# fdrmrc/fictitious_domain_AL_preconditioners

Measured on AMD Instinct MI355X. Metric: FGMRES iterations/sec to 1e-8 residual, 3D Stokes-immersed (AL-preconditioned), higher is better.
Workload: dtype f64

## Files before the change

### fictitious_domain_al_preconditioners_amd/csrc/alfd.hip

```cpp

#include <hip/hip_runtime.h>
#include <rccl/rccl.h>

#include <algorithm>
#include <atomic>
#include <chrono>
#include <cmath>
#include <cstdio>
#include <cstdlib>
#include <cstring>
#include <memory>
#include <climits>
#include <condition_variable>
#include <functional>
#include <limits>
#include <mutex>
#include <string>
#include <thread>
#include <unordered_set>
#include <vector>

#include "alfd/alfd.h"
#include "kernels.hpp"
#include "kernels_vs.hpp"
// ... 157 lines not shown
  alfd_host_alltoallv_fn host_alltoallv = nullptr;
  void *host_user = nullptr;
  std::vector<char> host_send, host_recv;
  std::vector<std::vector<int64_t>> part;
  int nblocks = 0;
  int64_t n[ALFD_MAX_BLOCKS] = {0, 0, 0};
  int64_t off[ALFD_MAX_BLOCKS + 1] = {0, 0, 0, 0};
  int64_t nmax = 0;
  int64_t diag_cap = 0;
  DevCsr mat[ALFD_NSLOTS + 1];
  double *diag[ALFD_NDIAGS] = {nullptr, nullptr};
  int64_t diag_n[ALFD_NDIAGS] = {0, 0};
  alfd_config cfg;
  bool configured = false, is_setup = false;
  double *sc = nullptr;
  double *sc_host = nullptr;
  double *partial = nullptr;
  int64_t pstride = 0;
  double *gather = nullptr;
  double *dinv_aug = nullptr, *dA = nullptr, *s_aug = nullptr;
  double *dinv_a22 = nullptr, *dinv_aug2 = nullptr;
  double lam_max[7] = {0, 0, 0, 0, 0, 0, 0};
  double *dinv_k = nullptr;
  double *dinv_m = nullptr, *m_tmp = nullptr, *m_tmp2 = nullptr;
  double *n_r = nullptr, *n_z = nullptr, *n_p = nullptr, *n_Ap = nullptr;
  double *n_sc = nullptr, *n_sc_host = nullptr, *n_partial = nullptr, *n_gather = nullptr;
  int64_t mass_its = 0;
  int n_owner = 0;
  double *gd_bx = nullptr, *gd_q = nullptr;
  int nmp_group = 16;
  int nmp_host_stepped = 0;
  struct Spectrum {
    DevCsr own_Cs, own_Cts;
    DevCsr *Cs = nullptr, *Cts = nullptr;
    int64_t m = 0;
    double *t = nullptr, *ones = nullptr, *x = nullptr, *coef = nullptr, *linf = nullptr;
    int64_t coef_cap = 0;
    std::vector<void *> owned;
    std::vector<double> alpha, beta;
    bool have = false;
  } spec;
  int spec_group = 16;
  int spec_host_stepped = 0;
  HostCsr h_M, h_K;
  struct Hierarchy {
    std::vector<int32_t> agg[ALFD_MAX_LEVELS];
    std::vector<double> wgt[ALFD_MAX_LEVELS];
    int64_t ncoarse[ALFD_MAX_LEVELS] = {0, 0, 0, 0, 0, 0, 0, 0};
    HostCsr P[ALFD_MAX_LEVELS];
    DevCsr inv;
    std::vector<MlLevel> ml;
    TailTable *tail_tab = nullptr;
    bool built_partitioned = false;
    void clear_input() {
      for (int l = 0; l < ALFD_MAX_LEVELS; ++l) agg[l].clear(), wgt[l].clear(), P[l] = HostCsr(), ncoarse[l] = 0;
      built_partitioned = false;
    }
  } hier[2];
  struct Patch {
    bool on = false;
    int64_t m = 0, mpad = 0;
    DevCsr Ass, As, Ats, Cs, Cts;
    int32_t *S = nullptr;
    double *dinv = nullptr, *rS = nullptr, *zS = nullptr, *uS = nullptr, *eS = nullptr, *cd = nullptr,
           *cres = nullptr, *ctmp = nullptr, *rr = nullptr;
    double lmax = 0;
    uint8_t *tail_mask = nullptr;
    bool rep = false;
    int64_t m_loc = 0, piece = 1, lam_piece = 1;
    std::vector<int64_t> soff;
    DevCsr Cts_loc, Ctg;
    double *send = nullptr, *stage = nullptr, *lam_send = nullptr, *lam_stage = nullptr, *loc = nullptr;
  } patch;
  struct StrengthGraph {
    bool have = false, on_device = false;
    int64_t n_nodes = 0, node0 = 0;
    std::vector<int64_t> gp;
    std::vector<int32_t> gc, fixed;
    std::vector<double> gw, d;
  } sg;
  int ml_rep_level = -1;
  bool dots_replicated = false;
  int64_t ml_rep_threshold = 300000;
  int ml_fuse = 1;
  int ml_tail_rows = 0;
  int ml_gpu_galerkin = 1;
  double *g_w = nullptr, *g_tlam = nullptr;
  std::vector<int64_t> ml_coff[ALFD_MAX_LEVELS];
  const int64_t *up_col_offsets = nullptr;
  bool up_local_only = false;
  DevCsr rat_mat;
  double *rt_r = nullptr, *rt_z = nullptr, *rt_p = nullptr, *rt_Ap = nullptr, *rt_x = nullptr;
  double *rt_dinv = nullptr, *rt_partial = nullptr, *rt_scb = nullptr, *rt_coef = nullptr;
  double *rt_scb_host = nullptr;
  int64_t rational_its = 0;
  int64_t wmax = 0;
  std::vector<void *> ws_allocs;
  double *w_r = nullptr, *w_z = nullptr, *w_p = nullptr, *w_Ap = nullptr;
  double *c_d = nullptr, *c_res = nullptr, *c_tmp = nullptr;
  double *t_lam = nullptr;
  double *q_tmp = nullptr, *rhs_tmp = nullptr;
  double *V = nullptr, *Z = nullptr, *xb = nullptr, *bb = nullptr, *io = nullptr;
  double *st_in = nullptr, *st_out = nullptr;
  double lambda_max = 0, lambda_min = 0;
  int64_t inner_its = 0, mp_its = 0;
  int64_t inner_its_op[3] = {0, 0, 0};
  int inner_failures = 0, precond_applications = 0;
  std::vector<double> history;
  int timing = 0;
  std::vector<TimedLaunch> timed;
  double t_ms[ALFD_T_NCLASSES] = {0, 0, 0, 0};
  int64_t t_launches[ALFD_T_NCLASSES] = {0, 0, 0, 0};
  double t_bytes[ALFD_T_NCLASSES] = {0, 0, 0, 0};
  double t_fbytes[ALFD_T_NCLASSES] = {0, 0, 0, 0};
  double setup_s[ALFD_SETUP_NPHASES] = {0, 0, 0, 0, 0, 0, 0, 0};
  bool upload_since_setup = false;
  std::vector<void *> allocs;
  int spmv_stream_R = 2, spmv_stream_U = 8, spmv_nt = 0, spmv_grid_mult = 8;
  int spmv_group_R = 4, spmv_group_U = 4;
  bool vi_off = false;
  int vi_rows_R = 4, vi_rows_J = 2;
  int vi_xcd = 0;
  int vi_levels = 1;
  int vi_batched = 1;
  int win_RB_vi = 96;
  int win_vi = 1;
  int win_short_scale = 2;
  int vs_enable = 1, vs_NW = 4, vs_RB = 96, vs_xcd = 0, vs_share = 1, vs_wide = 1;
  int vs_lds_base_ok = -1;
  std::vector<int64_t> rb_ptr[ALFD_NSLOTS + 1];
  std::vector<int32_t> rb_rows[ALFD_NSLOTS + 1];
  int win_short_min_blocks = 256;
  int win_min_blocks = 256;
  int win_enable = 1, win_RB = 96, win_maxW = 4096, win_gap = 8, win_xcd = 0;
  int64_t ntot() const { return off[nblocks]; }
};

struct alfd_local_group {
  int n = 0;
  std::mutex mu;
  std::condition_variable cv;
  int arrived = 0;
  long generation = 0;
  std::vector<const void *> buf;
  std::vector<const int64_t *> off;
  void barrier() {
    std::unique_lock<std::mutex> lk(mu);
    const long g = generation;
    if (++arrived == n) {
      arrived = 0;
      ++generation;
      cv.notify_all();
    } else {
      cv.wait(lk, [&] { return generation != g; });
    }
  }
};

namespace alfd {

static int comm_allgather(alfd_ctx *ctx, const void *send, void *recv, size_t bytes) {
  if (ctx->local) {
    alfd_local_group *g = ctx->local;
    HIPC(hipStreamSynchronize(ctx->stream));
    g->buf[ctx->rank] = send;
    g->barrier();
    for (int p = 0; p < g->n; ++p)
// ... 107 lines not shown
}

static inline int grid_for_rows(int64_t nrows, int L) {
  const int64_t groups = (nrows + (kBlock / L) - 1) / (kBlock / L);
  return (int)std::max<int64_t>(1, std::min<int64_t>(groups, 256 * 8));
}

struct Timer {
  alfd_ctx *ctx;
  int cls;
  hipEvent_t a = nullptr, b = nullptr;
  bool on;
  Timer(alfd_ctx *c, int cl, double bytes, double fbytes = -1.0) : ctx(c), cls(cl) {
    on = ctx->timing >= 2 || (ctx->timing == 1 && cl == ALFD_T_SPMV_A);
    if (on) {
      hipEventCreate(&a);
      hipEventCreate(&b);
      hipEventRecord(a, ctx->stream);
      ctx->t_bytes[cls] += bytes;
      ctx->t_fbytes[cls] += fbytes < 0.0 ? bytes : fbytes;
      ctx->t_launches[cls]++;
    }
  }
  ~Timer() {
    if (on) {
      hipEventRecord(b, ctx->stream);
      ctx->timed.push_back({cls, a, b});
    }
  }
};

struct PhaseClock {
  alfd_ctx *ctx;
  int phase;
  std::chrono::steady_clock::time_point t0 = std::chrono::steady_clock::now();
  PhaseClock(alfd_ctx *c, int ph) : ctx(c), phase(ph) {}
  ~PhaseClock() {
    hipStreamSynchronize(ctx->stream);
    ctx->setup_s[phase] += std::chrono::duration<double>(std::chrono::steady_clock::now() - t0).count();
  }
};

static void flush_timers(alfd_ctx *ctx) {
  for (auto &t : ctx->timed) {
    hipEventSynchronize(t.b);
    float ms = 0;
    hipEventElapsedTime(&ms, t.a, t.b);
    ctx->t_ms[t.cls] += ms;
    hipEventDestroy(t.a);
    hipEventDestroy(t.b);
  }
  ctx->timed.clear();
}

template <int L>
static void launch_spmv_L(alfd_ctx *ctx, const DevCsr &m, const double *x, double *y, int epi, double alpha,
                          const double *d, double *y2) {
  const int grid = grid_for_rows(m.n_list, L);
  const double *xh = m.halo;
#define ALFD_SPMV(EPI, SP)                                                                          \
  hipLaunchKernelGGL((spmv_kernel<L, EPI, SP>), dim3(grid), dim3(kBlock), 0, ctx->stream, m.n_list, \
                     m.rp, m.col, m.val, m.rows, x, xh, m.n_local_cols, y, alpha, d, y2)
  if (m.sparse) {
    if (epi == 0) ALFD_SPMV(0, true);
    else if (epi == 1) ALFD_SPMV(1, true);
    else if (epi == 2) ALFD_SPMV(2, true);
    else ALFD_SPMV(3, true);
  } else {
    if (epi == 0) ALFD_SPMV(0, false);
    else if (epi == 1) ALFD_SPMV(1, false);
    else if (epi == 2) ALFD_SPMV(2, false);
    else ALFD_SPMV(3, false);
  }
#undef ALFD_SPMV
}

template <int R, int U, bool NT>
static void launch_stream(alfd_ctx *ctx, const DevCsr &m, const double *x, double *y, int epi, double alpha,
                          const double *d, double *y2) {
  const int64_t nbatches = (m.nrows + R - 1) / R;
  const int grid = (int)std::max<int64_t>(1, std::min<int64_t>((nbatches + 3) / 4, 256 * ctx->spmv_grid_mult));
#define ALFD_STREAM(EPI)                                                                              \
  hipLaunchKernelGGL((spmv_stream_kernel<R, U, EPI, NT>), dim3(grid), dim3(kBlock), 0, ctx->stream,   \
                     m.nrows, m.rp, m.col, m.val, x, m.halo, m.n_local_cols, y, alpha, d, y2)
  if (epi == 0) ALFD_STREAM(0);
  else if (epi == 1) ALFD_STREAM(1);
  else if (epi == 2) ALFD_STREAM(2);
  else ALFD_STREAM(3);
#undef ALFD_STREAM
}

template <bool NT>
static bool launch_stream_RU(alfd_ctx *ctx, const DevCsr &m, const double *x, double *y, int epi,
                             double alpha, const double *d, double *y2) {
  const int R = ctx->spmv_stream_R, U = ctx->spmv_stream_U;
#define ALFD_RU(RR, UU) \
  if (R == RR && U == UU) return launch_stream<RR, UU, NT>(ctx, m, x, y, epi, alpha, d, y2), true
  ALFD_RU(2, 2); ALFD_RU(2, 4); ALFD_RU(4, 2); ALFD_RU(4, 4); ALFD_RU(4, 8); ALFD_RU(8, 4); ALFD_RU(8, 8);
  ALFD_RU(1, 4); ALFD_RU(2, 8); ALFD_RU(8, 2);
#undef ALFD_RU
  return false;
}

template <int R, int U>
static void launch_window(alfd_ctx *ctx, const DevCsr &m, const double *x, double *y, int epi, double alpha,
                          const double *d, double *y2) {
  const size_t lds = (size_t)(m.win_maxW + (m.vi && !ctx->vi_off ? kDictMaxEntries : 0)) * sizeof(double);
#define ALFD_WIN(EPI, TAG)                                                                              \
  hipLaunchKernelGGL((spmv_window_kernel<R, U, EPI, TAG>), dim3((unsigned)m.win_nblocks), dim3(kBlock), \
                     lds, ctx->stream, m.nrows, m.win_RB, m.rp, m.col, m.lcol, m.val, m.blk_seg_begin,   \
                     m.blk_W, m.seg_col, m.seg_off, x, m.halo, m.n_local_cols, y, alpha, d, y2, ctx->win_xcd)
  const bool vi = m.vi && !ctx->vi_off;
  if (vi && ctx->vi_batched && m.vib_tab) {
#define ALFD_VIB(EPI, TAG)                                                                                    \
  hipLaunchKernelGGL((spmv_window_vib_kernel<EPI, TAG>), dim3((unsigned)m.win_nblocks), dim3(kBlock), lds,   \
                     ctx->stream, m.nrows, m.win_RB, m.rp, m.col, m.lcol, m.val, m.blk_seg_begin, m.blk_W,    \
                     m.seg_col, m.seg_off, x, m.halo, m.n_local_cols, y, alpha, d, y2, m.vidx, m.vidw,        \
                     m.blk_dict_off, m.blk_dict_n, m.dict, m.win_maxW, m.vib_tab, m.vib_cnt, m.vib_stride,    \
                     ctx->vi_xcd)
    if (m.tag == 0) {
      if (epi == 0) ALFD_VIB(0, 0);
      else if (epi == 1) ALFD_VIB(1, 0);
      else if (epi == 2) ALFD_VIB(2, 0);
      else ALFD_VIB(3, 0);
    } else {
      if (epi == 0) ALFD_VIB(0, 1);
      else if (epi == 1) ALFD_VIB(1, 1);
      else if (epi == 2) ALFD_VIB(2, 1);
      else ALFD_VIB(3, 1);
    }
#undef ALFD_VIB
    return;
  }
  if (vi && ctx->vi_rows_R > 0) {
    const int RR = ctx->vi_rows_R, JJ = ctx->vi_rows_J;
#define ALFD_VI(RV, JV, EPI)                                                                                  \
  hipLaunchKernelGGL((spmv_window_vi_kernel<RV, JV, EPI>), dim3((unsigned)m.win_nblocks), dim3(kBlock), lds,  \
                     ctx->stream, m.nrows, m.win_RB, m.rp, m.col, m.lcol, m.val, m.blk_seg_begin, m.blk_W,     \
                     m.seg_col, m.seg_off, x, m.halo, m.n_local_cols, y, alpha, d, y2, m.vidx, m.vidw, \
                     m.blk_dict_off, m.blk_dict_n, m.dict, m.win_maxW)
#define ALFD_VI_E(RV, JV)              \
  if (RR == RV && JJ == JV) {          \
    if (epi == 0) ALFD_VI(RV, JV, 0);  \
    else if (epi == 1) ALFD_VI(RV, JV, 1); \
    else if (epi == 2) ALFD_VI(RV, JV, 2); \
    else ALFD_VI(RV, JV, 3);           \
    return;                            \
  }
    ALFD_VI_E(4, 3) ALFD_VI_E(2, 4) ALFD_VI_E(4, 4)
    if (epi == 0) ALFD_VI(4, 2, 0);
    else if (epi == 1) ALFD_VI(4, 2, 1);
    else if (epi == 2) ALFD_VI(4, 2, 2);
    else ALFD_VI(4, 2, 3);
    return;
#undef ALFD_VI_E
#undef ALFD_VI
  }
  if (m.tag == 0) {
    if (epi == 0) ALFD_WIN(0, 0);
    else if (epi == 1) ALFD_WIN(1, 0);
    else if (epi == 2) ALFD_WIN(2, 0);
    else ALFD_WIN(3, 0);
  } else {
    if (epi == 0) ALFD_WIN(0, 1);
    else if (epi == 1) ALFD_WIN(1, 1);
    else if (epi == 2) ALFD_WIN(2, 1);
    else ALFD_WIN(3, 1);
  }
#undef ALFD_WIN
}

template <int L, int R, int U>
static void launch_window_group(alfd_ctx *ctx, const DevCsr &m, const double *x, double *y, int epi,
                                double alpha, const double *d, double *y2) {
  const size_t lds = (size_t)m.win_maxW * sizeof(double);
#define ALFD_WING(EPI, TAG)                                                                               \
  hipLaunchKernelGGL((spmv_window_group_kernel<L, R, U, EPI, TAG>), dim3((unsigned)m.win_nblocks),       \
                     dim3(kBlock), lds, ctx->stream, m.nrows, m.win_RB, m.rp, m.col, m.lcol, m.val,        \
                     m.blk_seg_begin, m.blk_W, m.seg_col, m.seg_off, x, m.halo, m.n_local_cols, y, alpha, \
                     d, y2)
  if (m.tag == 0) {
    if (epi == 0) ALFD_WING(0, 0);
    else if (epi == 1) ALFD_WING(1, 0);
    else if (epi == 2) ALFD_WING(2, 0);
    else ALFD_WING(3, 0);
  } else {
    if (epi == 0) ALFD_WING(0, 1);
    else if (epi == 1) ALFD_WING(1, 1);
    else if (epi == 2) ALFD_WING(2, 1);
    else ALFD_WING(3, 1);
  }
#undef ALFD_WING
}

template <int L>
static bool launch_window_group_RU(alfd_ctx *ctx, const DevCsr &m, const double *x, double *y, int epi,
                                   double alpha, const double *d, double *y2) {
  const int R = ctx->spmv_group_R, U = ctx->spmv_group_U;
#define ALFD_RU(RR, UU) \
  if (R == RR && U == UU) return launch_window_group<L, RR, UU>(ctx, m, x, y, epi, alpha, d, y2), true
  ALFD_RU(4, 4); ALFD_RU(2, 4); ALFD_RU(4, 2); ALFD_RU(8, 4); ALFD_RU(8, 2);
#undef ALFD_RU
  return false;
}

static bool launch_window_RU(alfd_ctx *ctx, const DevCsr &m, const double *x, double *y, int epi,
                             double alpha, const double *d, double *y2) {
  if (m.L == 32) return launch_window_group_RU<32>(ctx, m, x, y, epi, alpha, d, y2);
  if (m.L == 16) return launch_window_group_RU<16>(ctx, m, x, y, epi, alpha, d, y2);
  if (m.L == 8) return launch_window_group_RU<8>(ctx, m, x, y, epi, alpha, d, y2);
  if (m.L != 64) return false;
  const int R = ctx->spmv_stream_R, U = ctx->spmv_stream_U;
#define ALFD_RU(RR, UU) \
  if (R == RR && U == UU) return launch_window<RR, UU>(ctx, m, x, y, epi, alpha, d, y2), true
  ALFD_RU(1, 4); ALFD_RU(2, 4); ALFD_RU(2, 8); ALFD_RU(4, 2); ALFD_RU(4, 4); ALFD_RU(4, 8); ALFD_RU(8, 4);
  ALFD_RU(1, 8); ALFD_RU(1, 16); ALFD_RU(2, 16);
#undef ALFD_RU
  return false;
}


template <int L>
static void launch_vss(alfd_ctx *ctx, const DevCsr &m, const double *x, double *y, int epi, double alpha,
                       const double *d, double *y2) {
  const DevCsr::Vs &v = m.vs;
  const size_t lds = (size_t)kVsWinOff + (size_t)v.maxW * sizeof(double);
#define ALFD_VSS(EPI, TAG)                                                                                          \
  hipLaunchKernelGGL((spmv_vss_kernel<L, EPI, TAG>), dim3((unsigned)v.nb), dim3(256), lds, ctx->stream, v.stream, \
                     v.sb, v.tab, v.cnt, v.stride, v.seg_begin, v.blkW, v.seg_col, v.seg_off, v.doff, v.dn, v.dict, \
                     x, m.halo, m.n_local_cols, y, alpha, d, y2)
  if (m.tag == 0) {
    if (epi == 0) ALFD_VSS(0, 0);
    else if (epi == 1) ALFD_VSS(1, 0);
    else if (epi == 2) ALFD_VSS(2, 0);
    else ALFD_VSS(3, 0);
  } else {
    if (epi == 0) ALFD_VSS(0, 1);
    else if (epi == 1) ALFD_VSS(1, 1);
    else if (epi == 2) ALFD_VSS(2, 1);
    else ALFD_VSS(3, 1);
  }
#undef ALFD_VSS
}

static bool launch_vs(alfd_ctx *ctx, const DevCsr &m, const double *x, double *y, int epi, double alpha,
                      const double *d, double *y2, int64_t first_block = 0, int64_t n_blocks = -1) {
  const DevCsr::Vs &v = m.vs;
  if (ctx->vs_lds_base_ok < 0) {
    uint32_t *probe = nullptr, base = 1;
    if (hipMalloc((void **)&probe, sizeof(uint32_t)) == hipSuccess) {
      hipLaunchKernelGGL(vs_lds_base_probe_kernel, dim3(1), dim3(64), 4096, ctx->stream, probe);
      hipMemcpyAsync(&base, probe, sizeof(uint32_t), hipMemcpyDeviceToHost, ctx->stream);
      hipStreamSynchronize(ctx->stream);
      hipFree(probe);
    }
    ctx->vs_lds_base_ok = base == 0 ? 1 : 0;
    if (!ctx->vs_lds_base_ok)
      std::fprintf(stderr, "[alfd] dynamic LDS does not start at offset 0 (%u): batch-major SpMV formats disabled\n", base);
  }
  if (!ctx->vs_lds_base_ok) return false;
  if (v.L == 32) return launch_vss<32>(ctx, m, x, y, epi, alpha, d, y2), true;
  if (v.L == 16) return launch_vss<16>(ctx, m, x, y, epi, alpha, d, y2), true;
  if (v.L == 8) return launch_vss<8>(ctx, m, x, y, epi, alpha, d, y2), true;
  const int NW = ctx->vs_NW;
  const size_t lds = (size_t)(v.wide ? VsFmt<1>::kWinOff : VsFmt<0>::kWinOff) + (size_t)v.maxW * sizeof(double);
  if (n_blocks < 0) n_blocks = v.nb - first_block;
  if (n_blocks <= 0) return true;
  const unsigned grid = (unsigned)n_blocks;
  const int32_t base = (int32_t)first_block;
#define ALFD_VS_ARGS \
  v.stream, v.tab, v.stride, v.hdrb, v.segx, v.seg_stride, v.dict, x, m.halo, m.n_local_cols, y, alpha, d, y2, ctx->vs_xcd, base
#define ALFD_VS(EPI, NWV)                                                                                        \
  do {                                                                                                           \
    if (v.wide)                                     \
      hipLaunchKernelGGL((spmv_vs_kernel<EPI, 0, 4, 1>), dim3(grid), dim3(256), lds, ctx->stream,     \
                         ALFD_VS_ARGS);                                                                          \
    else if (m.tag == 0)                                                                                         \
      hipLaunchKernelGGL((spmv_vs_kernel<EPI, 0, NWV>), dim3(grid), dim3(64 * NWV), lds, ctx->stream, \
                         ALFD_VS_ARGS);                                                                          \
    else                \
      hipLaunchKernelGGL((spmv_vs_kernel<EPI, 1, 4>), dim3(grid), dim3(256), lds, ctx->stream,        \
                         ALFD_VS_ARGS);                                                                          \
  } while (0)
#define ALFD_VS_E(NWV)                  \
  do {                                  \
    if (epi == 0) ALFD_VS(0, NWV);      \
    else if (epi == 1) ALFD_VS(1, NWV); \
    else if (epi == 2) ALFD_VS(2, NWV); \
    else ALFD_VS(3, NWV);               \
  } while (0)
  if (NW == 8) ALFD_VS_E(8);
  else if (NW == 2) ALFD_VS_E(2);
  else ALFD_VS_E(4);
#undef ALFD_VS_E
#undef ALFD_VS
#undef ALFD_VS_ARGS
  return true;
}

static int halo_exchange(alfd_ctx *ctx, DevCsr &m, const double *x, hipStream_t st = nullptr);
static int spmv_launch_local(alfd_ctx *ctx, DevCsr &m, const double *x, double *y, int epi, double alpha, const double *d,
                             double *y2);

static int spmv_m(alfd_ctx *ctx, DevCsr &m, int cls, const double *x, double *y, int epi, double alpha = 0.0,
                  const double *d = nullptr, double *y2 = nullptr) {
  if (!m.present) return ctx->err = "matrix not set", ALFD_E_NOT_SETUP;
  const bool exchange = ctx->nranks > 1 && !m.rep && (ctx->local || ctx->host_alltoallv || m.n_halo > 0 || m.send_off.back() > 0);
  const bool overlap = exchange && (ctx->overlap_halo > 0 || (ctx->overlap_halo < 0 && (ctx->local || ctx->host_alltoallv))) && ctx->xstream && m.vs.on && m.vs.L == 64 && ctx->vs_enable && !ctx->vi_off &&
                       m.vs.nb_interior > 0 && !m.sparse && m.n_list > 0;
  if (overlap) {
    Timer tm(ctx, cls, m.algorithmic_bytes(), m.streamed_bytes(true, true));
    HIPC(hipEventRecord(ctx->ev_x, ctx->stream));
    if (!launch_vs(ctx, m, x, y, epi, alpha, d, y2, 0, m.vs.nb_interior)) return ctx->err = "batch-major launch failed", ALFD_E_HIP;
    HIPC(hipStreamWaitEvent(ctx->xstream, ctx->ev_x, 0));
    RC(halo_exchange(ctx, m, x, ctx->xstream));
    HIPC(hipEventRecord(ctx->ev_halo, ctx->xstream));
    HIPC(hipStreamWaitEvent(ctx->stream, ctx->ev_halo, 0));
    launch_vs(ctx, m, x, y, epi, alpha, d, y2, m.vs.nb_interior, m.vs.nb - m.vs.nb_interior);
    HIPC(hipGetLastError());
    return ALFD_OK;
  }
  if (exchange) RC(halo_exchange(ctx, m, x));
  if (m.sparse && epi != 1) {
    HIPC(hipMemsetAsync(y, 0, m.nrows * sizeof(double), ctx->stream));
    if (epi == 3) HIPC(hipMemsetAsync(y2, 0, m.nrows * sizeof(double), ctx->stream));
  }
  if (m.n_list == 0) return ALFD_OK;
  Timer tm(ctx, cls, m.algorithmic_bytes(), m.streamed_bytes(!ctx->vi_off, ctx->vs_enable != 0 && !ctx->vi_off));
  return spmv_launch_local(ctx, m, x, y, epi, alpha, d, y2);
}

static int spmv_launch_local(alfd_ctx *ctx, DevCsr &m, const double *x, double *y, int epi, double alpha, const double *d,
                             double *y2) {
  if (m.vs.on && ctx->vs_enable && !ctx->vi_off && launch_vs(ctx, m, x, y, epi, alpha, d, y2)) {
    HIPC(hipGetLastError());
    return ALFD_OK;
  }
  if (m.win && launch_window_RU(ctx, m, x, y, epi, alpha, d, y2)) {
    HIPC(hipGetLastError());
    return ALFD_OK;
  }
  if (m.L == 64 && !m.sparse && ctx->spmv_stream_R > 0) {
    const bool ok = ctx->spmv_nt ? launch_stream_RU<true>(ctx, m, x, y, epi, alpha, d, y2)
                                 : launch_stream_RU<false>(ctx, m, x, y, epi, alpha, d, y2);
    if (ok) {
      HIPC(hipGetLastError());
      return ALFD_OK;
    }
  }
  switch (m.L) {
    case 4: launch_spmv_L<4>(ctx, m, x, y, epi, alpha, d, y2); break;
    case 8: launch_spmv_L<8>(ctx, m, x, y, epi, alpha, d, y2); break;
    case 16: launch_spmv_L<16>(ctx, m, x, y, epi, alpha, d, y2); break;
    case 32: launch_spmv_L<32>(ctx, m, x, y, epi, alpha, d, y2); break;
    default: launch_spmv_L<64>(ctx, m, x, y, epi, alpha, d, y2); break;
  }
  HIPC(hipGetLastError());
  return ALFD_OK;
}

static int pick_short_row_format(alfd_ctx *ctx, DevCsr &m) {
  if (!m.vs.on || m.vs.L == 64 || m.nnz < 20000000 || ctx->vi_off || !ctx->vs_enable || m.sparse) return ALFD_OK;
  double *x = nullptr, *y = nullptr;
  const int64_t nx = std::max<int64_t>(ctx->nranks > 1 && !m.rep ? m.n_local_cols : m.ncols, 1);
  HIPC(hipMalloc((void **)&x, nx * sizeof(double)));
  HIPC(hipMalloc((void **)&y, std::max<int64_t>(m.nrows, 1) * sizeof(double)));
  HIPC(hipMemsetAsync(x, 0, nx * sizeof(double), ctx->stream));
  hipEvent_t e0, e1;
  HIPC(hipEventCreate(&e0));
  HIPC(hipEventCreate(&e1));
  float t[2] = {0.f, 0.f};
  bool ok = true;
  for (int f = 0; f < 2 && ok; ++f) {
    for (int it = 0; it < 6 && ok; ++it) {
      if (it == 1) hipEventRecord(e0, ctx->stream);
      m.vs.on = f == 0;
      ok = spmv_launch_local(ctx, m, x, y, 0, 0.0, nullptr, nullptr) == ALFD_OK;
    }
    m.vs.on = true;
    hipEventRecord(e1, ctx->stream);
    hipEventSynchronize(e1);
    hipEventElapsedTime(&t[f], e0, e1);
  }
  hipEventDestroy(e0);
  hipEventDestroy(e1);
  hipFree(x);
  hipFree(y);
  HIPC(hipGetLastError());
  if (ok && t[1] < 0.9f * t[0]) {
    m.vs.on = false;
    if (ctx->cfg.log_level > 0 || std::getenv("ALFD_LOG_UPLOAD"))
      std::fprintf(stderr, "[alfd] short-row operator (%lld rows, %lld nnz): without the batch-major form %.3f ms, with it %.3f ms per launch "
                   "-> batch-major form dropped\n", (long long)m.nrows, (long long)m.nnz, t[1] / 5.0, t[0] / 5.0);
  }
  return ALFD_OK;
}

static int spmv(alfd_ctx *ctx, int slot, const double *x, double *y, int epi, double alpha = 0.0,
                const double *d = nullptr, double *y2 = nullptr) {
  DevCsr &m = ctx->mat[slot];
  if (!m.present) return ctx->err = "matrix slot " + std::to_string(slot) + " not set", ALFD_E_NOT_SETUP;
  return spmv_m(ctx, m, slot == ALFD_A ? ALFD_T_SPMV_A : ALFD_T_SPMV_OTHER, x, y, epi, alpha, d, y2);
}

static int finish_dots(alfd_ctx *ctx, int64_t nb, int count, int out, int fin) {
  if (ctx->nranks == 1 || ctx->dots_replicated) {
    hipLaunchKernelGGL(dot_final_kernel, dim3(count), dim3(kBlock), 0, ctx->stream, ctx->partial, nb,
                       ctx->pstride, ctx->sc, out, fin);
    HIPC(hipGetLastError());
    return ALFD_OK;
  }
  hipLaunchKernelGGL(dot_final_kernel, dim3(count), dim3(kBlock), 0, ctx->stream, ctx->partial, nb,
                     ctx->pstride, ctx->sc, (int)S_STAGE, (int)FIN_STORE);
  HIPC(hipGetLastError());
  RC(comm_allgather(ctx, ctx->sc + S_STAGE, ctx->gather, (size_t)count * sizeof(double)));
  const int tgt = fin == FIN_STORE ? out : (int)S_TMP;
  hipLaunchKernelGGL(rank_sum_kernel, dim3(1), dim3(64), 0, ctx->stream, ctx->gather, ctx->nranks, count,
                     ctx->sc, tgt);
  if (fin != FIN_STORE) {
    hipLaunchKernelGGL(dot_final_kernel, dim3(1), dim3(kBlock), 0, ctx->stream, ctx->sc + S_TMP,
                       (int64_t)1, (int64_t)0, ctx->sc, out, fin);
  }
  HIPC(hipGetLastError());
  return ALFD_OK;
}

static int dot_async(alfd_ctx *ctx, int64_t npad, const double *x, const double *y, int out,
                     int fin = FIN_STORE) {
  const int64_t nb = npad / kChunk;
  if (nb > 0) {
    Timer tm(ctx, ALFD_T_DOT, 16.0 * npad);
    hipLaunchKernelGGL(dot_partial_kernel, dim3((unsigned)nb), dim3(kBlock), 0, ctx->stream, x, y,
                       ctx->partial);
  }
  HIPC(hipGetLastError());
  return finish_dots(ctx, nb, 1, out, fin);
}

static int read_scalars(alfd_ctx *ctx, int first, int count) {
  hipLaunchKernelGGL(mirror_scalars_kernel, dim3(1), dim3(kBlock), 0, ctx->stream, ctx->sc + first,
                     ctx->sc_host + first, count);
  HIPC(hipGetLastError());
  HIPC(hipStreamSynchronize(ctx->stream));
  return ALFD_OK;
}

#define VEC_LAUNCH(kernel, npad, bytes_per_elem, ...)                                              \
  do {                                                                                             \
    if ((npad) > 0) {                                                                              \
      Timer tm__(ctx, ALFD_T_VEC, (double)(bytes_per_elem) * (double)(npad));                      \
      hipLaunchKernelGGL(kernel, dim3((unsigned)((npad) / kChunk)), dim3(kBlock), 0, ctx->stream,  \
                         __VA_ARGS__);                                                             \
    }                                                                                              \
  } while (0)

enum OpKind { OP_AUG = 0, OP_MP = 1, OP_A22 = 2, OP_AUG2 = 3, OP_K = 4, OP_MASS = 5, OP_CCT = 6 };

static inline int64_t op_npad(const alfd_ctx *ctx, int op) {
  if (op == OP_MASS || op == OP_CCT) return pad_chunk(ctx->n[ctx->nblocks - 1]);
  return (op == OP_AUG || op == OP_K) ? pad_chunk(ctx->n[0]) : op == OP_AUG2 ? ctx->off[2] : pad_chunk(ctx->n[1]);
}

static int winv_scale(alfd_ctx *ctx, double alpha, const double *src, double *dst);
static int nested_mp_solve(alfd_ctx *ctx, const double *b, double *x);

static inline bool gd_nested(const alfd_ctx *ctx) {
  return !ctx->cfg.grad_div_in_A && (ctx->cfg.variant == ALFD_AL_STOKES || ctx->cfg.variant == ALFD_AL_STOKES_DIAG);
}

static int op_apply(alfd_ctx *ctx, int op, const double *x, double *y, bool exact_w = false) {
  const double *w = ctx->diag[ALFD_INVW];
  switch (op) {
    case OP_AUG:
      RC(spmv(ctx, ALFD_A, x, y, 0));
      if (ctx->cfg.aug_assembled) return ALFD_OK;
      if (exact_w && ctx->cfg.w_inverse != ALFD_W_DIAGONAL) {
        RC(spmv(ctx, ALFD_C, x, ctx->t_lam, 0));
        RC(winv_scale(ctx, 1.0, ctx->t_lam, ctx->t_lam));
      } else {
        RC(spmv(ctx, ALFD_C, x, ctx->t_lam, 2, 0.0, w));
      }
      RC(spmv(ctx, ALFD_CT, ctx->t_lam, y, 1, ctx->cfg.gamma));
      if (!gd_nested(ctx)) return ALFD_OK;
      if (exact_w) {
        RC(spmv(ctx, ALFD_B, x, ctx->gd_bx, 0));
        RC(nested_mp_solve(ctx, ctx->gd_bx, ctx->gd_q));
      } else {
        RC(spmv(ctx, ALFD_B, x, ctx->gd_q, 2, 0.0, ctx->diag[ALFD_MP_LUMPED_INV]));
      }
      return spmv(ctx, ALFD_BT, ctx->gd_q, y, 1, ctx->cfg.gamma_grad_div);
    case OP_MASS:
      return spmv(ctx, ALFD_M, x, y, 0);
    case OP_CCT:
      RC(spmv_m(ctx, *ctx->spec.Cts, ALFD_T_SPMV_OTHER, x, ctx->spec.t, 0));
      return spmv_m(ctx, *ctx->spec.Cs, ALFD_T_SPMV_OTHER, ctx->spec.t, y, 0);
    case OP_MP:
      return spmv(ctx, ALFD_MP, x, y, 0);
    case OP_K:
      return spmv(ctx, ALFD_A, x, y, 0);
    case OP_A22:
      RC(spmv(ctx, ALFD_A2, x, y, 0));
      if (exact_w && ctx->cfg.w_inverse != ALFD_W_DIAGONAL) {
        RC(spmv(ctx, ALFD_M, x, ctx->t_lam, 0));
        RC(winv_scale(ctx, 1.0, ctx->t_lam, ctx->t_lam));
      } else {
        RC(spmv(ctx, ALFD_M, x, ctx->t_lam, 2, 0.0, w));
      }
      return spmv(ctx, ALFD_M, ctx->t_lam, y, 1, ctx->cfg.gamma2);
    default: {
      const double *x1 = x + ctx->off[1];
      double *y1 = y + ctx->off[1];
      const int64_t nlp = pad_chunk(ctx->n[2]);
      RC(spmv(ctx, ALFD_C, x, ctx->t_lam, 0));
      RC(spmv(ctx, ALFD_M, x1, ctx->t_lam, 1, -1.0));
      if (exact_w) RC(winv_scale(ctx, 1.0, ctx->t_lam, ctx->t_lam));
      else VEC_LAUNCH(pmul_scale_kernel, nlp, 24, 1.0, w, ctx->t_lam, ctx->t_lam);
      RC(spmv(ctx, ALFD_A, x, y, 0));
      RC(spmv(ctx, ALFD_CT, ctx->t_lam, y, 1, ctx->cfg.gamma));
      RC(spmv(ctx, ALFD_A2, x1, y1, 0));
      return spmv(ctx, ALFD_M, ctx->t_lam, y1, 1, -ctx->cfg.gamma2);
    }
  }
}

static const double *op_dinv(const alfd_ctx *ctx, int op) {
  return op == OP_AUG ? ctx->dinv_aug : op == OP_A22 ? ctx->dinv_a22 : op == OP_AUG2 ? ctx->dinv_aug2
         : op == OP_K ? ctx->dinv_k : op == OP_MASS ? ctx->dinv_m : ctx->diag[ALFD_MP_LUMPED_INV];
}

struct ChebCoef {
  double theta, delta, sigma, rho;
  ChebCoef(double lmax, double ratio) {
    const double lmin = lmax / ratio;
    theta = 0.5 * (lmax + lmin), delta = 0.5 * (lmax - lmin);
    sigma = theta / delta;
    rho = 1.0 / sigma;
  }
  void step(double &c1, double &c2) {
    const double rho_new = 1.0 / (2.0 * sigma - rho);
    c1 = rho_new * rho, c2 = 2.0 * rho_new / delta;
    rho = rho_new;
  }
};

template <class Apply>
static int cheb_sweep(alfd_ctx *ctx, int64_t npad, const double *dinv, double lmax, double ratio, int degree, double *cd,
                      double *cres, double *ctmp, const double *r, double *z, Apply apply) {
  ChebCoef k(lmax, ratio);
  VEC_LAUNCH(cheb_init_kernel, npad, degree > 1 ? 40 : 32, 1.0 / k.theta, dinv, r, cd, z, cres, degree > 1 ? 1 : 0);
  for (int j = 1; j < degree; ++j) {
    RC(apply(cd, ctmp));
    double c1, c2;
    k.step(c1, c2);
    VEC_LAUNCH(cheb_step_kernel, npad, 64, c1, c2, dinv, ctmp, cres, cd, z);
  }
  HIPC(hipGetLastError());
  return ALFD_OK;
}

static int cheb_apply(alfd_ctx *ctx, int op, const double *r, double *z, int64_t npad) {
  const int k = ctx->cfg.cheb_degree;
  if (k > 1) HIPC(hipMemsetAsync(ctx->c_tmp, 0, npad * sizeof(double), ctx->stream));
  return cheb_sweep(ctx, npad, op_dinv(ctx, op), ctx->lam_max[op], ctx->cfg.cheb_eig_ratio, k, ctx->c_d, ctx->c_res,
// ... 2401 lines not shown
    out.col.insert(out.col.end(), t_col[t].begin(), t_col[t].end());
    out.val.insert(out.val.end(), t_val[t].begin(), t_val[t].end());
  }
}

static int upload_matrix(alfd_ctx *ctx, int slot, int64_t nrows, int64_t ncols, const int64_t *rp,
                         const int32_t *col, const double *val);
static int upload_level(alfd_ctx *ctx, DevCsr &dst, const HostCsr &h) {
  static const int32_t no_col = 0;
  static const double no_val = 0;
  RC(upload_matrix(ctx, kScratchSlot, h.nrows, h.ncols, h.rp.data(), h.col.empty() ? &no_col : h.col.data(),
                   h.val.empty() ? &no_val : h.val.data()));
  csr_free(dst);
  dst = std::move(ctx->mat[kScratchSlot]);
  ctx->mat[kScratchSlot] = DevCsr();
  dst.tag = 1;
  return ALFD_OK;
}

struct AugOp {
  DevCsr *A = nullptr, *C = nullptr, *Ct = nullptr;
  int clsA = ALFD_T_SPMV_OTHER;
  const double *w = nullptr;
  double gamma = 0;
  double *tlam = nullptr;
  const uint8_t *mask = nullptr;
  int64_t npad = 0;
  const double *dinv = nullptr;
  double *cd = nullptr, *cres = nullptr, *ctmp = nullptr;
  double lmax = 0;
};

struct LevelView {
  AugOp op;
  double *r = nullptr, *z = nullptr, *t = nullptr;
  DevCsr *R = nullptr, *P = nullptr;
  double *rc = nullptr, *zc = nullptr;
};

static LevelView level_view(alfd_ctx *ctx, int h, int l) {
  MlLevel &L = ctx->hier[h].ml[l];
  const bool rep = h == 0 && ctx->ml_rep_level >= 0 && l >= ctx->ml_rep_level;
  LevelStore &S = rep ? L.rep : L.loc;
  LevelView V;
  AugOp &F = V.op;
  F.A = l > 0 ? &S.A : &ctx->mat[h == 0 ? ALFD_A : ALFD_A2];
  F.C = l > 0 ? &S.C : &ctx->mat[h == 0 ? ALFD_C : ALFD_M];
  F.Ct = l > 0 ? &S.Ct : &ctx->mat[h == 0 ? ALFD_CT : ALFD_M];
  F.clsA = l == 0 && h == 0 ? ALFD_T_SPMV_A : ALFD_T_SPMV_OTHER;
  F.w = rep ? ctx->g_w : ctx->diag[ALFD_INVW];
  F.gamma = h == 0 ? ctx->cfg.gamma : ctx->cfg.gamma2;
  F.tlam = rep ? ctx->g_tlam : ctx->t_lam;
  F.mask = L.tail_mask;
  F.npad = S.npad;
  F.dinv = S.dinv;
  F.cd = S.cd, F.cres = S.cres, F.ctmp = S.ctmp;
  F.lmax = L.lmax;
  V.r = S.r, V.z = S.z, V.t = S.t;
  if (l + 1 < (int)ctx->hier[h].ml.size()) {
    MlLevel &M = ctx->hier[h].ml[l + 1];
    LevelStore &N = rep ? M.rep : M.loc;
    V.R = &N.R, V.P = &N.P;
    V.rc = N.r, V.zc = N.z;
  }
  return V;
}

static AugOp patch_aug(alfd_ctx *ctx) {
  alfd_ctx::Patch &Q = ctx->patch;
  AugOp F;
  F.A = &Q.Ass, F.C = &Q.Cs, F.Ct = &Q.Cts;
  F.w = Q.rep ? ctx->g_w : ctx->diag[ALFD_INVW];
  F.tlam = Q.rep ? ctx->g_tlam : ctx->t_lam;
  F.gamma = ctx->cfg.gamma;
  F.mask = Q.tail_mask;
  F.npad = Q.mpad;
  F.dinv = Q.dinv;
  F.cd = Q.cd, F.cres = Q.cres, F.ctmp = Q.ctmp;
  F.lmax = Q.lmax;
  return F;
}

static int fused_AC(alfd_ctx *ctx, const AugOp &F, const double *x, double *y) {
  RC(spmv_m(ctx, *F.A, F.clsA, x, y, 0));
  return spmv_m(ctx, *F.C, ALFD_T_SPMV_OTHER, x, F.tlam, 2, 0.0, F.w);
}

static int aug_apply(alfd_ctx *ctx, const AugOp &F, const double *x, double *y) {
  if (ctx->cfg.aug_assembled) return spmv_m(ctx, *F.A, F.clsA, x, y, 0);
  RC(fused_AC(ctx, F, x, y));
  return spmv_m(ctx, *F.Ct, ALFD_T_SPMV_OTHER, F.tlam, y, 1, F.gamma);
}

static int aug_lambda_max(alfd_ctx *ctx, const AugOp &F, int64_t n, int64_t goff, double *v, double *wv, double *lmax) {
  if (n > 0)
    hipLaunchKernelGGL(hash_vector_kernel, dim3((unsigned)((n + 255) / 256)), dim3(256), 0, ctx->stream, n, goff, v);
  double lam = 0;
  RC(power_lambda(ctx, F.npad, F.dinv, v, wv, [&](const double *x, double *y) { return aug_apply(ctx, F, x, y); }, &lam));
  *lmax = lam * ctx->cfg.cheb_safety;
  HIPC(hipMemsetAsync(v, 0, F.npad * sizeof(double), ctx->stream));
  HIPC(hipMemsetAsync(wv, 0, F.npad * sizeof(double), ctx->stream));
  return ALFD_OK;
}


static bool plain_form(const alfd_ctx *ctx, const DevCsr &m) {
  return m.present && !m.vs.on && !m.win && !(m.L == 64 && !m.sparse && ctx->spmv_stream_R > 0);
}

static bool fused_ok(const alfd_ctx *ctx, const AugOp &F) {
  return ctx->ml_fuse && ctx->nranks == 1 && !ctx->cfg.aug_assembled && !gd_nested(ctx) &&
         ctx->cfg.w_inverse == ALFD_W_DIAGONAL && F.mask && F.A->present && F.C->present && plain_form(ctx, *F.Ct);
}

static int aug_tail(alfd_ctx *ctx, const AugOp &F, int mode, const AugTailArgs &p, double vec_bytes) {
  const DevCsr &m = *F.Ct;
  const int nb_rows = m.n_list > 0 ? grid_for_rows(m.n_list, m.L) : 0;
  const unsigned grid = (unsigned)nb_rows + (unsigned)(F.npad / kChunk);
  if (grid == 0) return ALFD_OK;
  Timer tm(ctx, ALFD_T_SPMV_OTHER, m.algorithmic_bytes() + vec_bytes * (double)F.npad,
           m.streamed_bytes(false) + vec_bytes * (double)F.npad);
#define ALFD_TAIL(LL, MM)                                                                                         \
  hipLaunchKernelGGL((aug_tail_kernel<LL, MM>), dim3(grid), dim3(kBlock), 0, ctx->stream, m.n_list, m.rp, m.col,  \
                     m.val, m.sparse ? m.rows : (const int32_t *)nullptr, F.tlam, nb_rows, F.mask, p)
#define ALFD_TAIL_L(LL)                                      \
  switch (mode) {                                            \
    case TAIL_STEP: ALFD_TAIL(LL, TAIL_STEP); break;         \
    case TAIL_LAST: ALFD_TAIL(LL, TAIL_LAST); break;         \
    case TAIL_LAST_ADD: ALFD_TAIL(LL, TAIL_LAST_ADD); break; \
    case TAIL_RES: ALFD_TAIL(LL, TAIL_RES); break;           \
    case TAIL_RES_INIT: ALFD_TAIL(LL, TAIL_RES_INIT); break; \
    default: ALFD_TAIL(LL, TAIL_RES_INIT_ADD); break;        \
  }
  switch (m.L) {
    case 4: ALFD_TAIL_L(4) break;
    case 8: ALFD_TAIL_L(8) break;
    case 16: ALFD_TAIL_L(16) break;
    case 32: ALFD_TAIL_L(32) break;
    default: ALFD_TAIL_L(64) break;
  }
#undef ALFD_TAIL_L
#undef ALFD_TAIL
  HIPC(hipGetLastError());
  return ALFD_OK;
}

static int cheb_fused(alfd_ctx *ctx, const AugOp &F, int degree, double ratio, const double *r, double *z, double *zout,
                      bool have_init) {
  ChebCoef k(F.lmax, ratio);
  if (!have_init) VEC_LAUNCH(cheb_init_z_kernel, F.npad, 24, 1.0 / k.theta, F.dinv, r, z);
  for (int j = 1; j < degree; ++j) {
    RC(fused_AC(ctx, F, j == 1 ? z : F.cd, F.ctmp));
    AugTailArgs p;
    k.step(p.c1, p.c2);
    p.gamma = F.gamma;
    p.dinv = F.dinv, p.y = F.ctmp, p.rin = j == 1 ? r : F.cres, p.din = j == 1 ? z : F.cd;
    p.res = F.cres, p.d = F.cd, p.z = z, p.zout = zout;
    const bool last = j == degree - 1;
    RC(aug_tail(ctx, F, !last ? TAIL_STEP : zout ? TAIL_LAST_ADD : TAIL_LAST, p, last && zout ? 88.0 : 64.0));
  }
  HIPC(hipGetLastError());
  return ALFD_OK;
}

static int aug_cheb(alfd_ctx *ctx, const AugOp &F, int degree, double ratio, const double *r, double *z) {
  if (fused_ok(ctx, F)) return cheb_fused(ctx, F, degree, ratio, r, z, nullptr, false);
  return cheb_sweep(ctx, F.npad, F.dinv, F.lmax, ratio, degree, F.cd, F.cres, F.ctmp, r, z,
                    [&](const double *x, double *y) { return aug_apply(ctx, F, x, y); });
}

static int fused_residual(alfd_ctx *ctx, const AugOp &F, const double *r, double *t) {
  AugTailArgs p;
  p.gamma = F.gamma, p.y = t, p.rin = r, p.res = t;
  return aug_tail(ctx, F, TAIL_RES, p, 24.0);
}

static int fused_correct(alfd_ctx *ctx, const AugOp &F, int degree, double ratio, const double *r, double *t, double *zc,
                         double *zout) {
  AugTailArgs p;
  p.gamma = F.gamma, p.c1 = 1.0 / ChebCoef(F.lmax, ratio).theta;
  p.dinv = F.dinv, p.y = t, p.rin = r, p.res = t, p.z = zc, p.zout = zout;
  p.store_res = degree > 1;
  if (degree <= 1 && zout) return aug_tail(ctx, F, TAIL_RES_INIT_ADD, p, 24.0 + 32.0 + 24.0);
  RC(aug_tail(ctx, F, TAIL_RES_INIT, p, 24.0 + (degree > 1 ? 40.0 : 32.0)));
  return cheb_fused(ctx, F, degree, ratio, t, zc, zout, true);
}

static int build_tail_mask(alfd_ctx *ctx, const DevCsr &m, int64_t npad, uint8_t **mask) {
  *mask = nullptr;
  if (ctx->nranks > 1 || !m.present || npad == 0 || m.nrows > npad) return ALFD_OK;
  double *q = nullptr;
  RC(ws_alloc_zero(ctx, &q, npad / 8));
  *mask = reinterpret_cast<uint8_t *>(q);
  if (m.n_list > 0)
    hipLaunchKernelGGL(mark_rows_kernel, dim3((unsigned)((m.n_list + 255) / 256)), dim3(256), 0, ctx->stream, m.n_list,
                       m.sparse ? m.rows : (const int32_t *)nullptr, *mask);
  HIPC(hipGetLastError());
  return ALFD_OK;
}

static_assert(kTailMaxLevels == ALFD_MAX_LEVELS + 1, "TailTable holds every level of a hierarchy");

static bool tail_form(const DevCsr &m) { return m.present && !m.vs.on && !m.win; }

static TailCsr tail_csr(const DevCsr &m) {
  TailCsr t;
  t.rp = m.rp, t.col = m.col, t.val = m.val, t.rows = m.sparse ? m.rows : nullptr;
  t.n_list = m.n_list, t.nrows = m.nrows;
  t.L = m.L, t.sparse = m.sparse ? 1 : 0;
  return t;
}

static int build_tail_table(alfd_ctx *ctx) {
  const alfd_config &c = ctx->cfg;
  alfd_ctx::Hierarchy &H = ctx->hier[1];
  const int last = (int)H.ml.size() - 1;
  std::vector<TailTable> tab(1);
  TailTable &T = tab[0];
  std::memset(&T, 0, sizeof(T));
  T.nlev = last + 1;
  T.has_inv = H.inv.present ? 1 : 0;
  if (H.inv.present) T.inv = tail_csr(H.inv);
  for (int l = 1; l <= last; ++l) {
    const LevelView V = level_view(ctx, 1, l);
    TailLevel &F = T.lev[l];
    F.A = tail_csr(*V.op.A), F.C = tail_csr(*V.op.C), F.Ct = tail_csr(*V.op.Ct);
    if (l < last) F.R = tail_csr(*V.R), F.P = tail_csr(*V.P);
    F.dinv = V.op.dinv, F.w = V.op.w, F.tlam = V.op.tlam;
    F.r = V.r, F.z = V.z, F.t = V.t, F.cd = V.op.cd, F.cres = V.op.cres, F.ctmp = V.op.ctmp;
    F.gamma = V.op.gamma, F.npad = V.op.npad;
    F.degree = l == last ? c.ml_coarse_degree : c.ml_smooth_degree_coarse > 0 ? c.ml_smooth_degree_coarse : c.ml_smooth_degree;
    ChebCoef k(V.op.lmax, l == last ? c.ml_coarse_ratio : c.ml_smooth_ratio);
    F.inv_theta = 1.0 / k.theta;
    for (int j = 1; j < F.degree && j <= kTailMaxDegree; ++j) k.step(F.c1[j - 1], F.c2[j - 1]);
  }
  double *q = nullptr;
  RC(ws_alloc_zero(ctx, &q, (int64_t)((sizeof(TailTable) + 7) / 8)));
  H.tail_tab = reinterpret_cast<TailTable *>(q);
  HIPC(hipMemcpyAsync(H.tail_tab, &T, sizeof(TailTable), hipMemcpyHostToDevice, ctx->stream));
  HIPC(hipStreamSynchronize(ctx->stream));
  return ALFD_OK;
}

static bool tail_ok(alfd_ctx *ctx, int l, const double *r, const double *z) {
  const alfd_config &c = ctx->cfg;
  alfd_ctx::Hierarchy &H = ctx->hier[1];
  const int last = (int)H.ml.size() - 1;
  if (!H.tail_tab || l < 1 || H.ml[l].loc.n > ctx->ml_tail_rows || r != H.ml[l].loc.r || z != H.ml[l].loc.z) return false;
  if (ctx->nranks != 1 || c.aug_assembled || c.w_inverse != ALFD_W_DIAGONAL) return false;
  const int sdeg = c.ml_smooth_degree_coarse > 0 ? c.ml_smooth_degree_coarse : c.ml_smooth_degree;
  if (sdeg - 1 > kTailMaxDegree || (!H.inv.present && c.ml_coarse_degree - 1 > kTailMaxDegree)) return false;
  if (H.inv.present && !tail_form(H.inv)) return false;
  for (int j = l; j <= last; ++j) {
    const LevelStore &L = H.ml[j].loc;
    if (!tail_form(L.A) || !tail_form(L.C) || !tail_form(L.Ct)) return false;
    if (j > l && (!tail_form(L.R) || !tail_form(L.P))) return false;
  }
  return true;
}

static int allgather_pieces(alfd_ctx *ctx, const double *mine, const std::vector<int64_t> &offs, int64_t piece, double *send,
                            double *stage, double *whole) {
  const int64_t n_me = offs[ctx->rank + 1] - offs[ctx->rank];
  if (n_me > 0) HIPC(hipMemcpyAsync(send, mine, n_me * sizeof(double), hipMemcpyDeviceToDevice, ctx->stream));
  RC(comm_allgather(ctx, send, stage, (size_t)piece * sizeof(double)));
  for (int p = 0; p < ctx->nranks; ++p) {
    const int64_t np = offs[p + 1] - offs[p];
    if (np > 0)
      HIPC(hipMemcpyAsync(whole + offs[p], stage + (int64_t)p * piece, np * sizeof(double), hipMemcpyDeviceToDevice, ctx->stream));
  }
  return ALFD_OK;
}

static int ml_cycle(alfd_ctx *ctx, int h, int l, const double *r, double *z) {
  const alfd_config &c = ctx->cfg;
  alfd_ctx::Hierarchy &H = ctx->hier[h];
  const int last = (int)H.ml.size() - 1;
  if (h == 1 && ctx->ml_tail_rows > 0 && tail_ok(ctx, l, r, z)) {
    Timer tm(ctx, ALFD_T_SPMV_OTHER, 0.0);
    hipLaunchKernelGGL(ml_tail_kernel, dim3(1), dim3(kTailBlock), 0, ctx->stream, H.tail_tab, l);
    HIPC(hipGetLastError());
    return ALFD_OK;
  }
  const LevelView L = level_view(ctx, h, l);
  const AugOp &F = L.op;
  if (l == last) {
// ... 9 lines not shown
  } else {
    RC(aug_apply(ctx, F, z, L.t));
    VEC_LAUNCH(sub_from_kernel, F.npad, 24, r, L.t);
  }
  RC(spmv_m(ctx, *L.R, ALFD_T_SPMV_OTHER, L.t, L.rc, 0));
  if (h == 0 && l + 1 == ctx->ml_rep_level) {
    MlLevel &N = H.ml[l + 1];
    RC(allgather_pieces(ctx, N.loc.r, N.offs, N.maxpiece, N.send, N.stage, N.rep.r));
    RC(ml_cycle(ctx, h, l + 1, N.rep.r, N.rep.z));
    RC(spmv_m(ctx, N.loc.P, ALFD_T_SPMV_OTHER, N.P_global_cols ? N.rep.z : N.rep.z + N.offs[ctx->rank], z, 1, 1.0));
  } else {
    RC(ml_cycle(ctx, h, l + 1, L.rc, L.zc));
    RC(spmv_m(ctx, *L.P, ALFD_T_SPMV_OTHER, L.zc, z, 1, 1.0));
  }
  if (fuse) {
    RC(fused_AC(ctx, F, z, L.t));
    RC(fused_correct(ctx, F, sdeg, c.ml_smooth_ratio, r, L.t, L.r, z));
    return ALFD_OK;
  }
  RC(aug_apply(ctx, F, z, L.t));
  VEC_LAUNCH(sub_from_kernel, F.npad, 24, r, L.t);
  RC(aug_cheb(ctx, F, sdeg, c.ml_smooth_ratio, L.t, L.r));
  VEC_LAUNCH(axpy_kernel, F.npad, 24, (const double *)nullptr, 0, 1.0, L.r, z);
  HIPC(hipGetLastError());
  return ALFD_OK;
}

static int ml_apply_rep(alfd_ctx *ctx, const double *r, double *z) {
  alfd_ctx::Patch &Q = ctx->patch;
  const int64_t n0p = pad_chunk(ctx->n[0]);
  const unsigned gm = (unsigned)std::max<int64_t>(1, (Q.m_loc + 255) / 256);
  const bool pen = !ctx->cfg.aug_assembled;
  const int last = ctx->nblocks - 1;
  const int64_t s0 = Q.soff[ctx->rank];
  const AugOp F = patch_aug(ctx);
  const int pdeg = ctx->cfg.ml_patch_degree;
  const double pratio = ctx->cfg.ml_patch_ratio;
  if (Q.m_loc > 0) hipLaunchKernelGGL(gather_kernel, dim3(gm), dim3(256), 0, ctx->stream, Q.m_loc, Q.S, r, Q.loc);
  RC(allgather_pieces(ctx, Q.loc, Q.soff, Q.piece, Q.send, Q.stage, Q.rS));
  RC(aug_cheb(ctx, F, pdeg, pratio, Q.rS, Q.zS));
  VEC_LAUNCH(scale_copy_kernel, n0p, 16, 1.0, r, Q.rr);
  RC(spmv_m(ctx, Q.Ats, ALFD_T_SPMV_OTHER, Q.zS, Q.rr, 1, -1.0));
  if (pen) {
    RC(spmv_m(ctx, Q.Cs, ALFD_T_SPMV_OTHER, Q.zS, ctx->g_tlam, 2, 0.0, ctx->g_w));
    RC(spmv_m(ctx, Q.Ctg, ALFD_T_SPMV_OTHER, ctx->g_tlam, Q.rr, 1, -ctx->cfg.gamma));
  }
  RC(ml_cycle(ctx, 0, 0, Q.rr, z));
  if (Q.m_loc > 0) hipLaunchKernelGGL(scatter_add_kernel, dim3(gm), dim3(256), 0, ctx->stream, Q.m_loc, Q.S, Q.zS + s0, z);
  RC(spmv_m(ctx, Q.As, ALFD_T_SPMV_OTHER, z, Q.loc, 0));
  if (pen) {
    RC(spmv(ctx, ALFD_C, z, ctx->t_lam, 2, 0.0, ctx->diag[ALFD_INVW]));
    RC(allgather_pieces(ctx, ctx->t_lam, ctx->part[last], Q.lam_piece, Q.lam_send, Q.lam_stage, ctx->g_tlam));
    RC(spmv_m(ctx, Q.Cts_loc, ALFD_T_SPMV_OTHER, ctx->g_tlam, Q.loc, 1, ctx->cfg.gamma));
  }
  RC(allgather_pieces(ctx, Q.loc, Q.soff, Q.piece, Q.send, Q.stage, Q.uS));
  VEC_LAUNCH(sub_from_kernel, Q.mpad, 24, Q.rS, Q.uS);
  RC(aug_cheb(ctx, F, pdeg, pratio, Q.uS, Q.eS));
  if (Q.m_loc > 0) hipLaunchKernelGGL(scatter_add_kernel, dim3(gm), dim3(256), 0, ctx->stream, Q.m_loc, Q.S, Q.eS + s0, z);
  HIPC(hipGetLastError());
  return ALFD_OK;
}

static int ml_apply(alfd_ctx *ctx, const double *r, double *z) {
  alfd_ctx::Patch &Q = ctx->patch;
  if (!Q.on) return ml_cycle(ctx, 0, 0, r, z);
  if (Q.rep) return ml_apply_rep(ctx, r, z);
  const int64_t n0p = pad_chunk(ctx->n[0]);
  const unsigned gm = (unsigned)((Q.m + 255) / 256);
  const bool pen = !ctx->cfg.aug_assembled;
  const double *w = ctx->diag[ALFD_INVW];
  const AugOp F = patch_aug(ctx);
  const int pdeg = ctx->cfg.ml_patch_degree;
  const double pratio = ctx->cfg.ml_patch_ratio;
  hipLaunchKernelGGL(gather_kernel, dim3(gm), dim3(256), 0, ctx->stream, Q.m, Q.S, r, Q.rS);
  RC(aug_cheb(ctx, F, pdeg, pratio, Q.rS, Q.zS));
  VEC_LAUNCH(scale_copy_kernel, n0p, 16, 1.0, r, Q.rr);
  RC(spmv_m(ctx, Q.Ats, ALFD_T_SPMV_OTHER, Q.zS, Q.rr, 1, -1.0));
  if (pen) {
    RC(spmv_m(ctx, Q.Cs, ALFD_T_SPMV_OTHER, Q.zS, ctx->t_lam, 2, 0.0, w));
    RC(spmv(ctx, ALFD_CT, ctx->t_lam, Q.rr, 1, -ctx->cfg.gamma));
  }
  RC(ml_cycle(ctx, 0, 0, Q.rr, z));
  hipLaunchKernelGGL(scatter_add_kernel, dim3(gm), dim3(256), 0, ctx->stream, Q.m, Q.S, Q.zS, z);
  RC(spmv_m(ctx, Q.As, ALFD_T_SPMV_OTHER, z, Q.uS, 0));
  if (fused_ok(ctx, F)) {
    RC(spmv(ctx, ALFD_C, z, ctx->t_lam, 2, 0.0, w));
    RC(fused_correct(ctx, F, pdeg, pratio, Q.rS, Q.uS, Q.eS, nullptr));
  } else {
    if (pen) {
      RC(spmv(ctx, ALFD_C, z, ctx->t_lam, 2, 0.0, w));
      RC(spmv_m(ctx, Q.Cts, ALFD_T_SPMV_OTHER, ctx->t_lam, Q.uS, 1, ctx->cfg.gamma));
    }
    VEC_LAUNCH(sub_from_kernel, Q.mpad, 24, Q.rS, Q.uS);
    RC(aug_cheb(ctx, F, pdeg, pratio, Q.uS, Q.eS));
  }
  hipLaunchKernelGGL(scatter_add_kernel, dim3(gm), dim3(256), 0, ctx->stream, Q.m, Q.S, Q.eS, z);
  HIPC(hipGetLastError());
  return ALFD_OK;
}

static void spgemm_host(const HostCsr &A, const HostCsr &Pm, HostCsr &out) {
  const int64_t nrows = A.nrows, nc = Pm.ncols;
  const int T = (int)std::max<int64_t>(1, std::min<int64_t>(std::min(16u, std::max(1u, std::thread::hardware_concurrency())),
                                                           (nrows + 4095) / 4096));
  std::vector<std::vector<int32_t>> t_cnt(T), t_col(T);
  std::vector<std::vector<double>> t_val(T);
  std::vector<std::thread> th;
  for (int t = 0; t < T; ++t)
    th.emplace_back([&, t]() {
      const int64_t i0 = nrows * t / T, i1 = nrows * (t + 1) / T;
      std::vector<int64_t> stamp(nc, -1);
      std::vector<double> acc(nc, 0.0);
      std::vector<int32_t> touched;
      t_cnt[t].reserve(i1 - i0);
      for (int64_t i = i0; i < i1; ++i) {
        touched.clear();
        for (int64_t k = A.rp[i]; k < A.rp[i + 1]; ++k) {
          const double a = A.val[k];
          const int64_t j = A.col[k];
          for (int64_t e = Pm.rp[j]; e < Pm.rp[j + 1]; ++e) {
            const int32_t J = Pm.col[e];
            if (stamp[J] != i) {
              stamp[J] = i;
              acc[J] = std::fma(a, Pm.val[e], 0.0);
              touched.push_back(J);
            } else {
              acc[J] = std::fma(a, Pm.val[e], acc[J]);
            }
          }
        }
        std::sort(touched.begin(), touched.end());
        t_cnt[t].push_back((int32_t)touched.size());
        for (int32_t J : touched) {
          t_col[t].push_back(J);
          t_val[t].push_back(acc[J]);
        }
      }
    });
  for (auto &x : th) x.join();
  out.nrows = nrows;
  out.ncols = nc;
  out.rp.assign(1, 0);
  out.rp.reserve(nrows + 1);
  int64_t total = 0;
  for (int t = 0; t < T; ++t) total += (int64_t)t_col[t].size();
  out.col.clear();
  out.val.clear();
  out.col.reserve(total);
  out.val.reserve(total);
  for (int t = 0; t < T; ++t) {
    for (int32_t c : t_cnt[t]) out.rp.push_back(out.rp.back() + c);
    out.col.insert(out.col.end(), t_col[t].begin(), t_col[t].end());
    out.val.insert(out.val.end(), t_val[t].begin(), t_val[t].end());
    std::vector<int32_t>().swap(t_col[t]);
    std::vector<double>().swap(t_val[t]);
  }
}

static void extract_host(const HostCsr &A, const std::vector<int32_t> &rows, const int32_t *colmap, int64_t ncols,
                         bool full_rows, HostCsr &out) {
  out.nrows = full_rows ? A.nrows : (int64_t)rows.size();
  out.ncols = ncols;
  out.rp.assign(out.nrows + 1, 0);
  out.col.clear();
  out.val.clear();
  int64_t next = 0;
  for (size_t q = 0; q < rows.size(); ++q) {
    const int64_t i = rows[q], orow = full_rows ? i : (int64_t)q;
    for (; next <= orow; ++next) out.rp[next] = (int64_t)out.col.size();
    for (int64_t k = A.rp[i]; k < A.rp[i + 1]; ++k) {
      const int32_t c = colmap ? colmap[A.col[k]] : A.col[k];
      if (c < 0) continue;
      out.col.push_back(c);
      out.val.push_back(A.val[k]);
    }
// ... 2247 lines not shown
    HIPC(hipMemcpyAsync(blocks[b], dev + ctx->off[b], ctx->n[b] * sizeof(double), hipMemcpyDeviceToHost,
                        ctx->stream));
  HIPC(hipStreamSynchronize(ctx->stream));
  return ALFD_OK;
}

static void reset_stats(alfd_ctx *ctx) {
  ctx->inner_its = ctx->mp_its = 0;
  ctx->inner_its_op[0] = ctx->inner_its_op[1] = ctx->inner_its_op[2] = 0;
  ctx->inner_failures = ctx->precond_applications = 0;
  ctx->rational_its = 0;
  ctx->mass_its = 0;
}
static void fill_result(alfd_ctx *ctx, alfd_result *res, int status) {
  res->status = status;
  res->inner_iterations = ctx->inner_its;
  res->mp_iterations = ctx->mp_its;
  res->inner_failures = ctx->inner_failures;
  res->precond_applications = ctx->precond_applications;
  res->lambda_max = ctx->lambda_max;
  res->rational_iterations = ctx->rational_its;
  res->mass_iterations = ctx->mass_its;
}

}

#define CHECK_CTX()                       \
  if (!ctx) return ALFD_E_INVALID;        \
  if (hipSetDevice(ctx->device) != hipSuccess) return ctx->err = "hipSetDevice failed", ALFD_E_HIP
#define CHECK_SETUP() \
  if (!ctx->is_setup) return ctx->err = "alfd_setup not called", ALFD_E_NOT_SETUP

extern "C" {

int alfd_abi_version(void) { return ALFD_ABI_VERSION; }

const char *alfd_strerror(int s) {
  switch (s) {
    case ALFD_OK: return "ok";
    case ALFD_E_INVALID: return "invalid argument";
    case ALFD_E_HIP: return "HIP runtime error";
    case ALFD_E_NO_CONVERGENCE_OUTER: return "FGMRES: no convergence (SolverControl::NoConvergence)";
    case ALFD_E_NO_CONVERGENCE_INNER: return "inner CG: no convergence (SolverControl::NoConvergence)";
    case ALFD_E_BREAKDOWN: return "breakdown (NaN residual)";
    case ALFD_E_NOT_SETUP: return "context not set up";
    case ALFD_E_COMM: return "RCCL error";
    case ALFD_E_UNSUPPORTED: return "not implemented";
    default: return "unknown status";
  }
}

const char *alfd_last_error(alfd_ctx_t ctx) { return ctx ? ctx->err.c_str() : "null context"; }

int alfd_create(alfd_ctx_t *out, int device_id) {
  if (!out) return ALFD_E_INVALID;
  *out = nullptr;
  int ndev = 0;
  if (hipGetDeviceCount(&ndev) != hipSuccess || ndev <= 0 || device_id < 0 || device_id >= ndev)
    return ALFD_E_HIP;
  if (hipSetDevice(device_id) != hipSuccess) return ALFD_E_HIP;
  alfd_ctx *ctx = new alfd_ctx;
  ctx->device = device_id;
  if (hipStreamCreateWithFlags(&ctx->xstream, hipStreamNonBlocking) != hipSuccess ||
      hipEventCreateWithFlags(&ctx->ev_x, hipEventDisableTiming) != hipSuccess ||
      hipEventCreateWithFlags(&ctx->ev_halo, hipEventDisableTiming) != hipSuccess)
    ctx->xstream = nullptr;
  if (const char *e = std::getenv("ALFD_SPMV_OVERLAP_HALO")) ctx->overlap_halo = std::atoi(e);
  if (hipStreamCreateWithFlags(&ctx->stream, hipStreamNonBlocking) != hipSuccess) {
    delete ctx;
    return ALFD_E_HIP;
  }
  alfd_default_config(&ctx->cfg, ALFD_AL_STOKES);
  if (const char *e = std::getenv("ALFD_SPMV_STREAM_R")) ctx->spmv_stream_R = std::atoi(e);
  if (const char *e = std::getenv("ALFD_SPMV_STREAM_U")) ctx->spmv_stream_U = std::atoi(e);
  if (const char *e = std::getenv("ALFD_SPMV_NT")) ctx->spmv_nt = std::atoi(e);
  if (const char *e = std::getenv("ALFD_SPMV_GRID")) ctx->spmv_grid_mult = std::max(1, std::atoi(e));
  if (const char *e = std::getenv("ALFD_SPMV_WINDOW")) ctx->win_enable = std::atoi(e);
  if (const char *e = std::getenv("ALFD_SPMV_WINDOW_RB")) ctx->win_RB = std::max(4, std::atoi(e));
  if (const char *e = std::getenv("ALFD_SPMV_WINDOW_MIN_BLOCKS")) ctx->win_min_blocks = std::max(1, std::atoi(e));
  if (const char *e = std::getenv("ALFD_SPMV_WINDOW_SHORT_MIN_BLOCKS")) ctx->win_short_min_blocks = std::max(1, std::atoi(e));
  if (const char *e = std::getenv("ALFD_SPMV_WINDOW_MAXW")) ctx->win_maxW = std::min(16384, std::max(256, std::atoi(e)));
  if (const char *e = std::getenv("ALFD_ML_REPLICATE")) ctx->ml_rep_threshold = std::atoll(e);
  if (const char *e = std::getenv("ALFD_ML_GPU_GALERKIN")) ctx->ml_gpu_galerkin = std::atoi(e);
  if (const char *e = std::getenv("ALFD_ML_FUSE")) ctx->ml_fuse = std::atoi(e) != 0;
  if (const char *e = std::getenv("ALFD_SPMV_VI_LEVELS")) ctx->vi_levels = std::atoi(e);
  if (const char *e = std::getenv("ALFD_SPMV_BATCH_MAJOR")) ctx->vs_enable = std::atoi(e);
  if (const char *e = std::getenv("ALFD_SPMV_BATCH_MAJOR_ROWS")) ctx->vs_RB = std::max(4, std::min(kVsMaxRows, std::atoi(e)));
  if (const char *e = std::getenv("ALFD_SPMV_VI_XCD")) ctx->vi_xcd = std::atoi(e);
  if (const char *e = std::getenv("ALFD_SPMV_VI_BATCHED")) ctx->vi_batched = std::atoi(e);
  if (const char *e = std::getenv("ALFD_SPMV_WINDOW_RB_VI")) ctx->win_RB_vi = std::atoi(e);
  if (const char *e = std::getenv("ALFD_SPMV_VI_R")) ctx->vi_rows_R = std::atoi(e);
  if (const char *e = std::getenv("ALFD_SPMV_VI_J")) ctx->vi_rows_J = std::atoi(e);
  if (const char *e = std::getenv("ALFD_SPMV_VALUE_INDEX")) ctx->win_vi = std::atoi(e);
  if (const char *e = std::getenv("ALFD_SPMV_GROUP_R")) ctx->spmv_group_R = std::atoi(e);
  if (const char *e = std::getenv("ALFD_SPMV_GROUP_U")) ctx->spmv_group_U = std::atoi(e);
  if (const char *e = std::getenv("ALFD_SPMV_WINDOW_SHORT")) ctx->win_short_scale = std::max(0, std::atoi(e));
  if (const char *e = std::getenv("ALFD_SPMV_WINDOW_GAP")) ctx->win_gap = std::max(1, std::atoi(e));
  if (const char *e = std::getenv("ALFD_SPMV_WINDOW_XCD")) ctx->win_xcd = std::atoi(e);
  *out = ctx;
  return ALFD_OK;
}

int alfd_destroy(alfd_ctx_t ctx) {
  if (!ctx) return ALFD_E_INVALID;
  hipSetDevice(ctx->device);
  hipStreamSynchronize(ctx->stream);
  flush_timers(ctx);
  free_levels(ctx);
  spectrum_release(ctx);
  csr_free(ctx->rat_mat);
  for (DevCsr &m : ctx->mat) csr_free(m);
  for (void *p : ctx->ws_allocs) hipFree(p);
  for (void *p : ctx->allocs) hipFree(p);
  if (ctx->sc_host) hipHostFree(ctx->sc_host);
  if (ctx->n_sc_host) hipHostFree(ctx->n_sc_host);
  if (ctx->rt_scb_host) hipHostFree(ctx->rt_scb_host);
  if (ctx->nccl) ncclCommDestroy(ctx->nccl);
  if (ctx->xstream) hipStreamDestroy(ctx->xstream);
  if (ctx->ev_x) hipEventDestroy(ctx->ev_x);
  if (ctx->ev_halo) hipEventDestroy(ctx->ev_halo);
  hipStreamDestroy(ctx->stream);
  delete ctx;
  return ALFD_OK;
}

int alfd_comm_unique_id(void *id_out, size_t bytes) {
  static_assert(sizeof(ncclUniqueId) <= ALFD_UNIQUE_ID_BYTES, "unique id size");
  if (!id_out || bytes < sizeof(ncclUniqueId)) return ALFD_E_INVALID;
  ncclUniqueId id;
  if (ncclGetUniqueId(&id) != ncclSuccess) return ALFD_E_COMM;
  std::memset(id_out, 0, bytes);
  std::memcpy(id_out, &id, sizeof(id));
  return ALFD_OK;
}

int alfd_comm_init(alfd_ctx_t ctx, int rank, int nranks, const void *id, size_t bytes) {
  CHECK_CTX();
  if (nranks < 1 || rank < 0 || rank >= nranks) return ALFD_E_INVALID;
  ctx->rank = rank;
  ctx->nranks = nranks;
  if (nranks == 1) return ALFD_OK;
  if (!id || bytes < sizeof(ncclUniqueId)) return ALFD_E_INVALID;
  ncclUniqueId uid;
  std::memcpy(&uid, id, sizeof(uid));
  if (ncclCommInitRank(&ctx->nccl, nranks, uid, rank) != ncclSuccess)
    return ctx->err = "ncclCommInitRank failed", ALFD_E_COMM;
  if (rank == 0) {
    int v = 0;
    if (ncclGetVersion(&v) == ncclSuccess) std::fprintf(stderr, "[alfd] RCCL version %d, %d ranks\n", v, nranks);
  }
  return ALFD_OK;
}

int alfd_local_group_create(int nranks, alfd_local_group **out) {
  if (!out || nranks < 1) return ALFD_E_INVALID;
  alfd_local_group *g = new alfd_local_group;
  g->n = nranks;
  g->buf.assign(nranks, nullptr);
  g->off.assign(nranks, nullptr);
  *out = g;
  return ALFD_OK;
}

int alfd_local_group_destroy(alfd_local_group *g) {
  if (!g) return ALFD_E_INVALID;
  delete g;
  return ALFD_OK;
// ... 974 lines not shown
                                                                    : fgmres(ctx, res);
  hipStreamSynchronize(ctx->stream);
  res->solve_seconds = std::chrono::duration<double>(std::chrono::steady_clock::now() - t0).count();
  flush_timers(ctx);
  fill_result(ctx, res, rc);
  return rc;
}

int alfd_download_solution(alfd_ctx_t ctx, double *const *x) {
  CHECK_CTX();
  CHECK_SETUP();
  if (!x) return ALFD_E_INVALID;
  return to_host(ctx, ctx->xb, x);
}

int alfd_solve(alfd_ctx_t ctx, const double *const *rhs, double *const *x, alfd_result *res) {
  CHECK_CTX();
  CHECK_SETUP();
  if (!rhs || !x || !res) return ALFD_E_INVALID;
  RC(alfd_upload_rhs(ctx, rhs, x));
  const int rc = alfd_solve_resident(ctx, res);
  const int rc2 = alfd_download_solution(ctx, x);
  return rc != ALFD_OK ? rc : rc2;
}

int alfd_get_history(alfd_ctx_t ctx, double *out, int32_t capacity, int32_t *count) {
  if (!ctx) return ALFD_E_INVALID;
  if (count) *count = (int32_t)ctx->history.size();
  if (out)
    for (int32_t i = 0; i < capacity && i < (int32_t)ctx->history.size(); ++i) out[i] = ctx->history[i];
  return ALFD_OK;
}

int alfd_spmv(alfd_ctx_t ctx, int slot, const double *x, double *y, int mode, double alpha) {
  CHECK_CTX();
  if (slot < 0 || slot >= ALFD_NSLOTS || !ctx->mat[slot].present) return ALFD_E_INVALID;
  if (!x || !y || (mode != 0 && mode != 1)) return ALFD_E_INVALID;
  const DevCsr &m = ctx->mat[slot];
  const int64_t nx = ctx->nranks > 1 ? (int64_t)m.n_local_cols : m.ncols;
  double *dx = nullptr, *dy = nullptr;
  HIPC(hipMalloc((void **)&dx, std::max<int64_t>(nx, 1) * sizeof(double)));
  HIPC(hipMalloc((void **)&dy, std::max<int64_t>(m.nrows, 1) * sizeof(double)));
  HIPC(hipMemcpyAsync(dx, x, nx * sizeof(double), hipMemcpyHostToDevice, ctx->stream));
  HIPC(hipMemcpyAsync(dy, y, m.nrows * sizeof(double), hipMemcpyHostToDevice, ctx->stream));
  const int rc = spmv(ctx, slot, dx, dy, mode, alpha);
  if (rc == ALFD_OK) {
    HIPC(hipMemcpyAsync(y, dy, m.nrows * sizeof(double), hipMemcpyDeviceToHost, ctx->stream));
    HIPC(hipStreamSynchronize(ctx->stream));
  }
  hipFree(dx);
  hipFree(dy);
  return rc;
}

int alfd_spmv_scaled(alfd_ctx_t ctx, int slot, const double *x, const double *d, double *y, double *y2) {
  CHECK_CTX();
  if (slot < 0 || slot >= ALFD_NSLOTS || !ctx->mat[slot].present) return ALFD_E_INVALID;
  if (!x || !d || !y || y2 == y) return ALFD_E_INVALID;
  const DevCsr &m = ctx->mat[slot];
  const int64_t nx = ctx->nranks > 1 ? (int64_t)m.n_local_cols : m.ncols;
  const size_t rows = std::max<int64_t>(m.nrows, 1) * sizeof(double), nb = m.nrows * sizeof(double);
  double *dx = nullptr, *dd = nullptr, *dy = nullptr, *dy2 = nullptr;
  HIPC(hipMalloc((void **)&dx, std::max<int64_t>(nx, 1) * sizeof(double)));
  HIPC(hipMalloc((void **)&dd, rows));
  HIPC(hipMalloc((void **)&dy, rows));
  if (y2) HIPC(hipMalloc((void **)&dy2, rows));
  HIPC(hipMemcpyAsync(dx, x, nx * sizeof(double), hipMemcpyHostToDevice, ctx->stream));
  HIPC(hipMemcpyAsync(dd, d, nb, hipMemcpyHostToDevice, ctx->stream));
  HIPC(hipMemcpyAsync(dy, y, nb, hipMemcpyHostToDevice, ctx->stream));
  if (y2) HIPC(hipMemcpyAsync(dy2, y2, nb, hipMemcpyHostToDevice, ctx->stream));
  const int rc = spmv(ctx, slot, dx, dy, y2 ? 3 : 2, 0.0, dd, dy2);
  if (rc == ALFD_OK) {
    HIPC(hipMemcpyAsync(y, dy, nb, hipMemcpyDeviceToHost, ctx->stream));
    if (y2) HIPC(hipMemcpyAsync(y2, dy2, nb, hipMemcpyDeviceToHost, ctx->stream));
    HIPC(hipStreamSynchronize(ctx->stream));
  }
  hipFree(dx);
  hipFree(dd);
  hipFree(dy);
  hipFree(dy2);
  return rc;
}

int alfd_inner_prec_apply(alfd_ctx_t ctx, int op, const double *r, double *z) {
  CHECK_CTX();
  CHECK_SETUP();
  if (!r || !z) return ALFD_E_INVALID;
  const int v = ctx->cfg.variant;
  int kind = -1;
  if (op == ALFD_INNER_OP_AUG &&
      (v == ALFD_AL2 || v == ALFD_AL_STOKES || v == ALFD_AL_STOKES_DIAG || v == ALFD_AL_ELL_MODIFIED))
    kind = OP_AUG;
  else if (op == ALFD_INNER_OP_A22 && v == ALFD_AL_ELL_MODIFIED)
    kind = OP_A22;
  else if (op == ALFD_INNER_OP_AUG2 && v == ALFD_AL_ELL_IDEAL)
    kind = OP_AUG2;
  if (kind < 0)
    return ctx->err = "alfd_inner_prec_apply: the configured variant has no such inner operator", ALFD_E_INVALID;
  const int b0 = kind == OP_A22 ? 1 : 0, b1 = kind == OP_AUG2 ? 1 : b0;
  const int64_t npad = op_npad(ctx, kind);
  double *dr = ctx->st_in + ctx->off[b0], *dz = ctx->st_out + ctx->off[b0];
  HIPC(hipMemsetAsync(ctx->st_in, 0, ctx->ntot() * sizeof(double), ctx->stream));
  HIPC(hipMemsetAsync(ctx->st_out, 0, ctx->ntot() * sizeof(double), ctx->stream));
  int64_t at = 0;
  for (int b = b0; b <= b1; ++b) {
    HIPC(hipMemcpyAsync(ctx->st_in + ctx->off[b], r + at, ctx->n[b] * sizeof(double), hipMemcpyHostToDevice,
                        ctx->stream));
    at += ctx->n[b];
  }
  const int prec = ctx->cfg.inner_prec;
  if (prec == ALFD_PREC_IDENTITY) {
    HIPC(hipMemcpyAsync(dz, dr, npad * sizeof(double), hipMemcpyDeviceToDevice, ctx->stream));
  } else if (prec == ALFD_PREC_JACOBI) {
    VEC_LAUNCH(jacobi_dot_kernel, npad, 24, op_dinv(ctx, kind), dr, dz, ctx->partial);
    HIPC(hipGetLastError());
  } else if (prec == ALFD_PREC_MULTILEVEL && ml_covers(ctx, kind)) {
    RC(ml_prec(ctx, kind, dr, dz));
  } else {
    RC(cheb_apply(ctx, kind, dr, dz, npad));
  }
  at = 0;
  for (int b = b0; b <= b1; ++b) {
    HIPC(hipMemcpyAsync(z + at, ctx->st_out + ctx->off[b], ctx->n[b] * sizeof(double), hipMemcpyDeviceToHost,
                        ctx->stream));
    at += ctx->n[b];
  }
  HIPC(hipStreamSynchronize(ctx->stream));
  return ALFD_OK;
}

int alfd_dot(alfd_ctx_t ctx, int64_t n, const double *x, const double *y, double *result) {
  CHECK_CTX();
  if (n < 0 || !x || !y || !result) return ALFD_E_INVALID;
  const int64_t npad = pad_chunk(std::max<int64_t>(n, 1));
  double *dx = nullptr, *dy = nullptr, *part = nullptr, *sc = nullptr;
  HIPC(hipMalloc((void **)&dx, npad * sizeof(double)));
  HIPC(hipMalloc((void **)&dy, npad * sizeof(double)));
  HIPC(hipMalloc((void **)&part, (npad / kChunk) * sizeof(double)));
  HIPC(hipMalloc((void **)&sc, kNumScalars * sizeof(double)));
  HIPC(hipMemsetAsync(dx, 0, npad * sizeof(double), ctx->stream));
  HIPC(hipMemsetAsync(dy, 0, npad * sizeof(double), ctx->stream));
  HIPC(hipMemcpyAsync(dx, x, n * sizeof(double), hipMemcpyHostToDevice, ctx->stream));
  HIPC(hipMemcpyAsync(dy, y, n * sizeof(double), hipMemcpyHostToDevice, ctx->stream));
  hipLaunchKernelGGL(dot_partial_kernel, dim3((unsigned)(npad / kChunk)), dim3(kBlock), 0, ctx->stream, dx,
                     dy, part);
  hipLaunchKernelGGL(dot_final_kernel, dim3(1), dim3(kBlock), 0, ctx->stream, part, npad / kChunk,
                     (int64_t)0, sc, (int)S_TMP, (int)FIN_STORE);
  HIPC(hipGetLastError());
  HIPC(hipMemcpyAsync(result, sc + S_TMP, sizeof(double), hipMemcpyDeviceToHost, ctx->stream));
  HIPC(hipStreamSynchronize(ctx->stream));
  hipFree(dx);
  hipFree(dy);
  hipFree(part);
  hipFree(sc);
  return ALFD_OK;
}

int alfd_host_halo_plan(int64_t nnz, const int32_t *col, const int64_t *col_offsets, int nranks, int rank,
                        int32_t *col_local, int32_t *halo_globals, int64_t halo_capacity, int64_t *n_halo,
                        int64_t *recv_off) {
  if (nnz < 0 || nranks < 1 || rank < 0 || rank >= nranks || !col_offsets || !col_local || !n_halo || !recv_off ||
      (nnz > 0 && !col))
    return ALFD_E_INVALID;
  std::vector<int32_t> hal;
  host_halo_plan(nnz, col, col_offsets, nranks, rank, col_local, hal, recv_off);
  *n_halo = (int64_t)hal.size();
// ... 468 lines not shown
  for (int64_t i = 0; i < nrows; ++i) rows_out[i] = key[i].second;
  *n_blocks_out = nb;
  return ALFD_OK;
}

int alfd_host_permute_csr(int64_t nrows, const int64_t *rp, const int32_t *col, const double *val,
                          const int64_t *row_new_to_old, const int64_t *col_old_to_new, int64_t *orp, int32_t *ocol,
                          double *oval) {
  if (nrows < 0 || !rp || !orp || (rp[nrows] > 0 && (!col || !val || !ocol || !oval))) return ALFD_E_INVALID;
  orp[0] = 0;
  for (int64_t r = 0; r < nrows; ++r) {
    const int64_t src = row_new_to_old ? row_new_to_old[r] : r;
    if (src < 0 || src >= nrows) return ALFD_E_INVALID;
    orp[r + 1] = orp[r] + (rp[src + 1] - rp[src]);
  }
  if (orp[nrows] != rp[nrows]) return ALFD_E_INVALID;
  const int T = (int)std::max<int64_t>(1, std::min<int64_t>(std::min(16u, std::max(1u, std::thread::hardware_concurrency())),
                                                           (nrows + 8191) / 8192));
  std::vector<std::thread> th;
  for (int t = 0; t < T; ++t)
    th.emplace_back([&, t]() {
      std::vector<std::pair<int32_t, double>> row;
      for (int64_t r = nrows * t / T; r < nrows * (t + 1) / T; ++r) {
        const int64_t src = row_new_to_old ? row_new_to_old[r] : r;
        const int64_t k0 = rp[src], len = rp[src + 1] - k0, o0 = orp[r];
        if (!col_old_to_new) {
          for (int64_t k = 0; k < len; ++k) ocol[o0 + k] = col[k0 + k], oval[o0 + k] = val[k0 + k];
          continue;
        }
        row.resize(len);
        for (int64_t k = 0; k < len; ++k) row[k] = {(int32_t)col_old_to_new[col[k0 + k]], val[k0 + k]};
        std::sort(row.begin(), row.end(), [](const auto &x, const auto &y) { return x.first < y.first; });
        for (int64_t k = 0; k < len; ++k) ocol[o0 + k] = row[k].first, oval[o0 + k] = row[k].second;
      }
    });
  for (auto &x : th) x.join();
  return ALFD_OK;
}

int alfd_get_device_memory(alfd_ctx_t ctx, int64_t *free_bytes, int64_t *total_bytes) {
  CHECK_CTX();
  size_t f = 0, t = 0;
  HIPC(hipMemGetInfo(&f, &t));
  if (free_bytes) *free_bytes = (int64_t)f;
  if (total_bytes) *total_bytes = (int64_t)t;
  return ALFD_OK;
}

int alfd_set_tunable(alfd_ctx_t ctx, const char *name, int value) {
  if (!ctx || !name) return ALFD_E_INVALID;
  if (std::strcmp(name, "value_index") == 0) {
    ctx->vi_off = value == 0;
    if (value == 0) RC(ensure_window_plans(ctx));
    return ALFD_OK;
  }
  if (std::strcmp(name, "batch_major") == 0) {
    ctx->vs_enable = value != 0;
    if (value == 0) RC(ensure_window_plans(ctx));
    return ALFD_OK;
  }
  if (std::strcmp(name, "batch_major_share") == 0) {
    ctx->vs_share = value != 0;
    return ALFD_OK;
  }
  if (std::strcmp(name, "batch_major_wide") == 0) {
    ctx->vs_wide = value != 0;
    return ALFD_OK;
  }
  if (std::strcmp(name, "batch_major_waves") == 0) {
    if (value != 2 && value != 4 && value != 8) return ctx->err = "batch_major_waves: 2, 4 or 8", ALFD_E_INVALID;
    ctx->vs_NW = value;
    return ALFD_OK;
  }
  if (std::strcmp(name, "batch_major_rows") == 0) {
    if (value < 4 || value > kVsMaxRows) return ctx->err = "batch_major_rows: 4..250", ALFD_E_INVALID;
    ctx->vs_RB = value;
    return ALFD_OK;
  }
  if (std::strcmp(name, "batch_major_xcd") == 0) {
    ctx->vs_xcd = value != 0;
    return ALFD_OK;
  }
  if (std::strcmp(name, "ml_fuse") == 0) {
    ctx->ml_fuse = value != 0;
    return ALFD_OK;
  }
  if (std::strcmp(name, "ml_tail_rows") == 0) {
    if (value < 0) return ctx->err = "ml_tail_rows: >= 0", ALFD_E_INVALID;
    ctx->ml_tail_rows = value;
    return ALFD_OK;
  }
  if (std::strcmp(name, "nested_mp_group") == 0) {
    if (value < 1 || value > 1000) return ctx->err = "nested_mp_group: 1..1000", ALFD_E_INVALID;
    ctx->nmp_group = value;
    return ALFD_OK;
  }
  if (std::strcmp(name, "nested_mp_host_stepped") == 0) {
    ctx->nmp_host_stepped = value != 0;
    return ALFD_OK;
  }
  if (std::strcmp(name, "spectrum_group") == 0) {
    if (value < 1 || value > 1000) return ctx->err = "spectrum_group: 1..1000", ALFD_E_INVALID;
    ctx->spec_group = value;
    return ALFD_OK;
  }
  if (std::strcmp(name, "spectrum_host_stepped") == 0) {
    ctx->spec_host_stepped = value != 0;
    return ALFD_OK;
  }
  return ctx->err = std::string("unknown tunable ") + name, ALFD_E_INVALID;
}

int alfd_host_tridiagonal_extremes(int32_t k, const double *alpha, const double *beta, double *lambda_min,
                                   double *lambda_max) {
  return host_tridiagonal_extremes(k, alpha, beta, lambda_min, lambda_max);
}

int alfd_estimate_spectrum(alfd_ctx_t ctx, int op, const alfd_control *ctrl, alfd_spectrum *out) {
  CHECK_CTX();
  CHECK_SETUP();
  if (!out) return ALFD_E_INVALID;
  if (op != ALFD_SPECTRUM_CCT) return ctx->err = "alfd_estimate_spectrum: unknown operator", ALFD_E_INVALID;
  if (ctx->nranks > 1) return ctx->err = "alfd_estimate_spectrum: single rank only", ALFD_E_UNSUPPORTED;
  const int64_t nl = ctx->n[ctx->nblocks - 1];
  alfd_control c;
  if (ctrl) {
    c = *ctrl;
  } else {
    c.kind = ALFD_CTRL_ABS;
    c.max_steps = (int32_t)std::min<int64_t>(nl, INT32_MAX);
    c.tol = 1e-12;
    c.reduce = 0.0;
  }
  if (c.kind < ALFD_CTRL_ABS || c.kind > ALFD_CTRL_FIXED_ITERS || c.max_steps < 1)
    return ctx->err = "alfd_estimate_spectrum: bad control (max_steps >= 1)", ALFD_E_INVALID;
  if (nl < 1) return ctx->err = "alfd_estimate_spectrum: no multipliers", ALFD_E_INVALID;
  return estimate_spectrum(ctx, c, out);
}

int alfd_get_cg_coefficients(alfd_ctx_t ctx, double *alpha, double *beta, int32_t capacity, int32_t *count) {
  if (!ctx) return ALFD_E_INVALID;
  if (!ctx->spec.have) return ctx->err = "no spectrum estimate yet", ALFD_E_NOT_SETUP;
  const int32_t k = (int32_t)ctx->spec.alpha.size();
  if (count) *count = k;
  for (int32_t i = 0; i < capacity && i < k; ++i) {
    if (alpha) alpha[i] = ctx->spec.alpha[i];
    if (beta && i + 1 < k) beta[i] = ctx->spec.beta[i];
  }
  return ALFD_OK;
}

int alfd_constraint_residual(alfd_ctx_t ctx, const double *const *x_blocks, const double *g, double *linf) {
  CHECK_CTX();
  CHECK_SETUP();
  if (!x_blocks || !linf) return ALFD_E_INVALID;
  if (ctx->nranks > 1) return ctx->err = "alfd_constraint_residual: single rank only", ALFD_E_UNSUPPORTED;
  return constraint_residual(ctx, x_blocks, g, linf);
}

int alfd_set_row_blocks(alfd_ctx_t ctx, int slot, int64_t n_blocks, const int64_t *block_ptr, const int32_t *rows) {
  if (!ctx || slot < 0 || slot >= ALFD_NSLOTS) return ALFD_E_INVALID;
  ctx->rb_ptr[slot].clear();
  ctx->rb_rows[slot].clear();
  if (n_blocks <= 0 || !block_ptr || !rows) return ALFD_OK;
  if (block_ptr[0] != 0) return ctx->err = "alfd_set_row_blocks: block_ptr[0] must be 0", ALFD_E_INVALID;
  for (int64_t b = 0; b < n_blocks; ++b)
    if (block_ptr[b + 1] < block_ptr[b]) return ctx->err = "alfd_set_row_blocks: block_ptr must be monotone", ALFD_E_INVALID;
// ... 36 lines not shown
```

### fictitious_domain_al_preconditioners_amd/csrc/kernels.hpp

```cpp
#pragma once
#include <hip/hip_runtime.h>
#include <stdint.h>

namespace alfd {

constexpr int kBlock = 256;
constexpr int64_t kChunk = 4096;
constexpr int kMaxBasis = 64;

__device__ __forceinline__ double dpp_xor_mov(double v, int which) {
  int lo = __double2loint(v), hi = __double2hiint(v), rl, rh;
  if (which == 8) {
    rl = __builtin_amdgcn_update_dpp(0, lo, 0x128, 0xf, 0xf, true);
    rh = __builtin_amdgcn_update_dpp(0, hi, 0x128, 0xf, 0xf, true);
  } else if (which == 4) {
    rl = __builtin_amdgcn_update_dpp(0, lo, 0x104, 0xf, 0x5, false);
    rl = __builtin_amdgcn_update_dpp(rl, lo, 0x114, 0xf, 0xa, false);
    rh = __builtin_amdgcn_update_dpp(0, hi, 0x104, 0xf, 0x5, false);
    rh = __builtin_amdgcn_update_dpp(rh, hi, 0x114, 0xf, 0xa, false);
  } else if (which == 2) {
    rl = __builtin_amdgcn_update_dpp(0, lo, 0x4E, 0xf, 0xf, true);
    rh = __builtin_amdgcn_update_dpp(0, hi, 0x4E, 0xf, 0xf, true);
  } else {
    rl = __builtin_amdgcn_update_dpp(0, lo, 0xB1, 0xf, 0xf, true);
    rh = __builtin_amdgcn_update_dpp(0, hi, 0xB1, 0xf, 0xf, true);
  }
  return __hiloint2double(rh, rl);
}
__device__ __forceinline__ void swap32(double &a, double &b) {
  auto l = __builtin_amdgcn_permlane32_swap((unsigned)__double2loint(a), (unsigned)__double2loint(b), false, false);
  auto h = __builtin_amdgcn_permlane32_swap((unsigned)__double2hiint(a), (unsigned)__double2hiint(b), false, false);
  a = __hiloint2double((int)h[0], (int)l[0]);
  b = __hiloint2double((int)h[1], (int)l[1]);
}
__device__ __forceinline__ void swap16(double &a, double &b) {
  auto l = __builtin_amdgcn_permlane16_swap((unsigned)__double2loint(a), (unsigned)__double2loint(b), false, false);
  auto h = __builtin_amdgcn_permlane16_swap((unsigned)__double2hiint(a), (unsigned)__double2hiint(b), false, false);
  a = __hiloint2double((int)h[0], (int)l[0]);
  b = __hiloint2double((int)h[1], (int)l[1]);
}
template <int L>
__device__ __forceinline__ double group_reduce(double v) {
  if (L >= 64) {
    double a = v, b = v;
    swap32(a, b);
    v = a + b;
  }
  if (L >= 32) {
    double p = v, q = v;
    swap16(p, q);
    v = p + q;
  }
  if (L >= 16) v = v + dpp_xor_mov(v, 8);
  if (L >= 8) v = v + dpp_xor_mov(v, 4);
  if (L >= 4) v = v + dpp_xor_mov(v, 2);
  if (L >= 2) v = v + dpp_xor_mov(v, 1);
  return v;
}

template <int N>
__device__ __forceinline__ double dpp_shl(double v) {
  const int lo = __double2loint(v), hi = __double2hiint(v);
  const int rl = __builtin_amdgcn_update_dpp(0, lo, 0x100 + N, 0xf, 0xf, true);
  const int rh = __builtin_amdgcn_update_dpp(0, hi, 0x100 + N, 0xf, 0xf, true);
  return __hiloint2double(rh, rl);
}
__device__ __forceinline__ double row16_tree(double v) {
  v = v + dpp_xor_mov(v, 8);
  v = v + dpp_shl<4>(v);
  v = v + dpp_shl<2>(v);
  v = v + dpp_shl<1>(v);
  return v;
}
__device__ __forceinline__ double reduce_rows4(double a0, double a1, double a2, double a3) {
  swap32(a0, a1);
  double p = a0 + a1;
  swap32(a2, a3);
  double q = a2 + a3;
  swap16(p, q);
  return row16_tree(p + q);
}
__device__ __forceinline__ double reduce_rows8(double a0, double a1, double a2, double a3, double a4, double a5,
                                               double a6, double a7, int lane) {
  swap32(a0, a1);
  double p01 = a0 + a1;
  swap32(a2, a3);
  double p23 = a2 + a3;
  swap32(a4, a5);
  double p45 = a4 + a5;
  swap32(a6, a7);
  double p67 = a6 + a7;
  swap16(p01, p23);
  double u = p01 + p23;
  swap16(p45, p67);
  double w = p45 + p67;
  u = u + dpp_xor_mov(u, 8);
  w = w + dpp_xor_mov(w, 8);
  double x = (lane & 8) ? w : u;
  x = x + dpp_shl<4>(x);
  x = x + dpp_shl<2>(x);
  x = x + dpp_shl<1>(x);
  return x;
}

template <int N>
__device__ __forceinline__ double dpp_shr(double v) {
  const int lo = __double2loint(v), hi = __double2hiint(v);
  const int rl = __builtin_amdgcn_update_dpp(0, lo, 0x110 + N, 0xf, 0xf, true);
  const int rh = __builtin_amdgcn_update_dpp(0, hi, 0x110 + N, 0xf, 0xf, true);
  return __hiloint2double(rh, rl);
}
__device__ __forceinline__ double reduce_rows16(double (&a)[16], int lane) {
  double p[8], u[4];
#pragma unroll
  for (int j = 0; j < 8; ++j) {
    swap32(a[2 * j], a[2 * j + 1]);
    p[j] = a[2 * j] + a[2 * j + 1];
  }
#pragma unroll
  for (int j = 0; j < 4; ++j) {
    swap16(p[2 * j], p[2 * j + 1]);
    u[j] = p[2 * j] + p[2 * j + 1];
    u[j] = u[j] + dpp_xor_mov(u[j], 8);
  }
  const bool h = (lane & 8) != 0;
  double x0 = h ? u[1] : u[0], x1 = h ? u[3] : u[2];
  x0 = x0 + dpp_shl<4>(x0);
  x1 = x1 + dpp_shr<4>(x1);
  double z = (lane & 4) ? x1 : x0;
  z = z + dpp_shl<2>(z);
  z = z + dpp_shl<1>(z);
  return z;
}

__device__ __forceinline__ double reduce_rows2(double a0, double a1) {
  swap32(a0, a1);
  double p = a0 + a1, q = p;
  swap16(p, q);
  return row16_tree(p + q);
}

__device__ __forceinline__ double block_reduce_256(double v, double *lds4) {
  v = group_reduce<64>(v);
  const int wave = threadIdx.x >> 6;
  if ((threadIdx.x & 63) == 0) lds4[wave] = v;
  __syncthreads();
  return (lds4[0] + lds4[1]) + (lds4[2] + lds4[3]);
}

template <int L, int EPI, bool SPARSE>
__global__ __launch_bounds__(kBlock) void spmv_kernel(int64_t nrows, const int64_t *__restrict__ rp,
                                                      const int32_t *__restrict__ col,
                                                      const double *__restrict__ val,
                                                      const int32_t *__restrict__ rows,
                                                      const double *__restrict__ x,
                                                      const double *__restrict__ x_halo, int32_t n_local,
                                                      double *__restrict__ y, double alpha,
                                                      const double *__restrict__ d,
                                                      double *__restrict__ y2) {
  constexpr int RPB = kBlock / L;
  const int lane = threadIdx.x % L;
  const int sub = threadIdx.x / L;
  const int64_t ngroups = (nrows + RPB - 1) / RPB;
  for (int64_t g = blockIdx.x; g < ngroups; g += gridDim.x) {
    const int64_t r = g * RPB + sub;
    if (r < nrows) {
      const int64_t k0 = rp[r], k1 = rp[r + 1];
      double acc = 0.0;
      for (int64_t k = k0 + lane; k < k1; k += L) {
        const int32_t c = col[k];
        const double xv = (c < n_local) ? x[c] : x_halo[c - n_local];
        acc = fma(val[k], xv, acc);
      }
      acc = group_reduce<L>(acc);
      if (lane == 0) {
        const int64_t ro = SPARSE ? (int64_t)rows[r] : r;
        if (EPI == 0)
          y[ro] = acc;
        else if (EPI == 1)
          y[ro] = fma(alpha, acc, y[ro]);
        else if (EPI == 2)
          y[ro] = d[ro] * acc;
        else {
          y[ro] = acc;
          y2[ro] = d[ro] * acc;
        }
      }
    }
  }
}

template <int R, int U, int EPI, bool NT>
__global__ __launch_bounds__(kBlock) void spmv_stream_kernel(
    int64_t nrows, const int64_t *__restrict__ rp, const int32_t *__restrict__ col,
    const double *__restrict__ val, const double *__restrict__ x, const double *__restrict__ x_halo,
    int32_t n_local, double *__restrict__ y, double alpha, const double *__restrict__ d,
    double *__restrict__ y2) {
  const int lane = threadIdx.x & 63;
  const int wave = __builtin_amdgcn_readfirstlane(threadIdx.x >> 6);
  const int64_t nbatches = (nrows + R - 1) / R;
  for (int64_t b = (int64_t)blockIdx.x * 4 + wave; b < nbatches; b += (int64_t)gridDim.x * 4) {
    const int64_t r0 = b * R;
    int64_t kb[R + 1];
#pragma unroll
    for (int i = 0; i <= R; ++i) kb[i] = rp[r0 + i < nrows ? r0 + i : nrows];
    const int64_t k_begin = kb[0];
    const int32_t n_batch = (int32_t)(kb[R] - k_begin);
    int32_t rel[R + 1];
#pragma unroll
    for (int i = 0; i <= R; ++i) rel[i] = (int32_t)(kb[i] - k_begin);
    double acc[R];
#pragma unroll
    for (int i = 0; i < R; ++i) acc[i] = 0.0;
    const int32_t *cb = col + k_begin;
    const double *vb = val + k_begin;
    for (int32_t base = 0; base < n_batch; base += 64 * U) {
      int32_t c[U];
      double v[U], xv[U];
#pragma unroll
      for (int u = 0; u < U; ++u) {
        const int32_t o = base + 64 * u + lane;
        if (o < n_batch) {
          c[u] = NT ? __builtin_nontemporal_load(cb + o) : cb[o];
          v[u] = NT ? __builtin_nontemporal_load(vb + o) : vb[o];
        } else {
          c[u] = -1;
          v[u] = 0.0;
        }
      }
#pragma unroll
      for (int u = 0; u < U; ++u) {
        xv[u] = 0.0;
        if (c[u] >= 0) xv[u] = (c[u] < n_local) ? x[c[u]] : x_halo[c[u] - n_local];
      }
#pragma unroll
      for (int u = 0; u < U; ++u) {
        const int32_t o = base + 64 * u + lane;
        if (c[u] >= 0) {
#pragma unroll
          for (int i = 0; i < R; ++i)
            if (o >= rel[i] && o < rel[i + 1]) acc[i] = fma(v[u], xv[u], acc[i]);
        }
      }
    }
#pragma unroll
    for (int i = 0; i < R; ++i) {
      const int64_t r = r0 + i;
      if (r < nrows) {
        const int dsh = rel[i] & 63;
        double s = __shfl(acc[i], (lane + dsh) & 63, 64);
        s = group_reduce<64>(s);
        if (lane == 0) {
          if (EPI == 0)
            y[r] = s;
          else if (EPI == 1)
            y[r] = fma(alpha, s, y[r]);
          else if (EPI == 2)
            y[r] = d[r] * s;
          else {
            y[r] = s;
            y2[r] = d[r] * s;
          }
        }
      }
    }
  }
}

template <int R, int U, int EPI, int TAG = 0>
__global__ __launch_bounds__(kBlock) void spmv_window_kernel(
    int64_t nrows, int32_t RB, const int64_t *__restrict__ rp, const int32_t *__restrict__ col,
    const uint16_t *__restrict__ lcol, const double *__restrict__ val,
    const int32_t *__restrict__ blk_seg_begin, const int32_t *__restrict__ blk_W,
    const int32_t *__restrict__ seg_col, const int32_t *__restrict__ seg_off,
    const double *__restrict__ x, const double *__restrict__ x_halo, int32_t n_local,
    double *__restrict__ y, double alpha, const double *__restrict__ d, double *__restrict__ y2,
    int xcd_remap) {
  extern __shared__ double xs[];
  const int lane = threadIdx.x & 63;
  const int wave = __builtin_amdgcn_readfirstlane(threadIdx.x >> 6);
  int64_t b = blockIdx.x;
  if (xcd_remap) {
    const int64_t nwg = gridDim.x, q = nwg / 8, rm = nwg % 8, xcd = b % 8, idx = b / 8;
    b = (xcd < rm ? xcd * (q + 1) : rm * (q + 1) + (xcd - rm) * q) + idx;
// ... 2070 lines not shown
```

### fictitious_domain_al_preconditioners_amd/csrc/kernels_vs.hpp

```cpp
#pragma once

namespace alfd {

constexpr int kVsMaxDict = 512;
constexpr int kVsDictOff = 0;
constexpr int kVsWinOff = kVsMaxDict * 8;
constexpr int kVsMaxRows = 250;
template <int WD>
struct VsFmt {
  static constexpr uint32_t kColMask = WD ? 0x3ff8u : 0x7ff8u;
  static constexpr int kDictShift = WD ? 11 : 12;
  static constexpr uint32_t kDictMask = WD ? 0x1ff8u : 0xff8u;
  static constexpr int kWinOff = WD ? 8192 : 4096;
  static constexpr int kCodeShift = WD ? 14 : 15;
  static constexpr int kMaxDict = WD ? 1024 : 512;
  static constexpr int kMaxSlots = WD ? 2048 : 4096;
};
constexpr int kVsMaxLen = 384;

__device__ __forceinline__ uint32_t vs_off(uint32_t d) { return d & 0xfffffu; }
__device__ __forceinline__ int32_t vs_len(uint32_t d) { return (int32_t)((d >> 20) & 0x1ffu); }
__device__ __forceinline__ int vs_cls(uint32_t d) { return (int)((d >> 29) & 7u); }

__device__ __forceinline__ double vs_lds_f64(uint32_t byte_off) {
// ... 6 lines not shown
}

struct VsWord3 {
  uint32_t x, y, z;
};

template <int NCH, int WD>
__device__ __forceinline__ void vs_batch(const int32_t (&rem)[4], int32_t maxrem, int lane,
                                         const uint8_t *__restrict__ fb, const char *sm, double (&acc)[4]) {
  VsWord3 w[NCH];
#pragma unroll
  for (int j = 0; j < NCH - 1; ++j) w[j] = *(const VsWord3 *)(fb + 768 * j + 12u * (uint32_t)lane);
  w[NCH - 1] = *(const VsWord3 *)(fb + 768 * (NCH - 1) + 12u * (uint32_t)(lane < maxrem ? lane : maxrem - 1));
#pragma unroll
  for (int j = 0; j < NCH; ++j) {
    double xv[4], v[4];
    const uint32_t f[4] = {w[j].x, __builtin_amdgcn_alignbit(w[j].y, w[j].x, 24),
                           __builtin_amdgcn_alignbit(w[j].z, w[j].y, 16), w[j].z >> 8};
#pragma unroll
    for (int i = 0; i < 4; ++i) {
      xv[i] = vs_lds_f64(VsFmt<WD>::kWinOff + (f[i] & VsFmt<WD>::kColMask));
      v[i] = vs_lds_f64(kVsDictOff + ((f[i] >> VsFmt<WD>::kDictShift) & VsFmt<WD>::kDictMask));
    }
#pragma unroll
    for (int i = 0; i < 4; ++i) asm volatile("" : "+v"(xv[i]), "+v"(v[i]));
#pragma unroll
    for (int i = 0; i < 4; ++i) {
      if (j == NCH - 1) {
        if (lane < rem[i]) acc[i] = fma(v[i], xv[i], acc[i]);
      } else {
        acc[i] = fma(v[i], xv[i], acc[i]);
      }
    }
  }
}

__device__ __forceinline__ void vs_shared_fetch(uint32_t d0, const uint8_t *__restrict__ sbase, int lane, uint32_t (&w)[6]) {
  const int cls = vs_cls(d0);
  const uint8_t *fb = sbase + 16u * (size_t)vs_off(d0);
  const int32_t rem = vs_len(d0) - 64 * (cls - 1);
  uint32_t l4 = 4u * (uint32_t)lane, r4 = 4u * (uint32_t)(lane < rem ? lane : rem - 1);
  asm volatile("" : "+v"(l4), "+v"(r4));
  w[0] = *(const uint32_t *)(fb + 256 * (cls - 1) + r4);
#pragma unroll
  for (int j = 0; j < 5; ++j)
    if (j < cls - 1) w[1 + j] = *(const uint32_t *)(fb + 256 * j + l4);
}

template <int NCH, int R, int WD>
__device__ __forceinline__ void vs_shared(int32_t rem, const int32_t (&sh)[R], int lane, const uint32_t (&w)[6],
                                          double (&acc)[R]) {
#pragma unroll
  for (int j = 0; j < NCH; ++j) {
    const uint32_t wj = j == NCH - 1 ? w[0] : w[1 + (j < 5 ? j : 0)];
    const uint32_t lc = wj & VsFmt<WD>::kColMask;
    double v = vs_lds_f64(kVsDictOff + ((wj >> VsFmt<WD>::kDictShift) & VsFmt<WD>::kDictMask));
    constexpr int G = R > 8 ? 4 : R;
#pragma unroll
    for (int g = 0; g < R; g += G) {
      double xv[G];
#pragma unroll
      for (int i = 0; i < G; ++i) xv[i] = vs_lds_f64(VsFmt<WD>::kWinOff + (uint32_t)((int32_t)lc + sh[g + i]));
#pragma unroll
      for (int i = 0; i < G; ++i) asm volatile("" : "+v"(xv[i]));
      if (g == 0) asm volatile("" : "+v"(v));
      if (j == NCH - 1) {
        if (lane < rem) {
          asm volatile("");
#pragma unroll
          for (int i = 0; i < G; ++i) acc[g + i] = fma(v, xv[i], acc[g + i]);
        }
      } else {
#pragma unroll
        for (int i = 0; i < G; ++i) acc[g + i] = fma(v, xv[i], acc[g + i]);
      }
      if (R > 8) {
#pragma unroll
        for (int i = 0; i < G; ++i) asm volatile("" : "+v"(acc[g + i]));
      }
    }
  }
}

template <int EPI, int TAG, int NW, int WD = 0>
__global__ __launch_bounds__(64 * NW) __attribute__((amdgpu_waves_per_eu(8, 8))) void spmv_vs_kernel(
    const uint8_t *__restrict__ stream, const uint64_t *__restrict__ tab, int32_t stride,
    const int32_t *__restrict__ hdrb, const int32_t *__restrict__ segx, int32_t seg_stride,
    const double *__restrict__ dict, const double *__restrict__ x, const double *__restrict__ x_halo,
    int32_t n_local, double *__restrict__ y, double alpha, const double *__restrict__ d, double *__restrict__ y2,
    int xcd_remap, int32_t block_base) {
  extern __shared__ double xs[];
  char *sm = (char *)xs;
  double *ds = (double *)(sm + kVsDictOff);
  double *xw = (double *)(sm + VsFmt<WD>::kWinOff);
  const int lane = threadIdx.x & 63;
  const int wave = __builtin_amdgcn_readfirstlane(threadIdx.x >> 6);
  int64_t b = blockIdx.x;
  if (xcd_remap) {
    const int64_t nwg = gridDim.x, q = nwg / 8, rm = nwg % 8, xcd = b % 8, idx = b / 8;
    b = (xcd < rm ? xcd * (q + 1) : rm * (q + 1) + (xcd - rm) * q) + idx;
  }
  b += block_base;
  const int32_t *hb = hdrb + 8 * b;
  const int32_t nbatch = hb[0], W = hb[1], nseg = hb[2], nd = hb[3], doff = hb[4];
  const uint8_t *sbase = stream + (int64_t)(((uint64_t)(uint32_t)hb[6] << 32) | (uint64_t)(uint32_t)hb[5]);
  const int32_t *sx = segx + 2 * b * (int64_t)seg_stride;
  const uint32_t *tb = (const uint32_t *)(tab + (int64_t)b * stride * 16);
  const int hl = lane & 31;
  auto hdr_at = [&](int32_t q) {
    uint32_t h4 = 4u * (uint32_t)hl;
    asm volatile("" : "+v"(h4));
    return *(const uint32_t *)((const char *)(tb + 32 * (int64_t)q) + h4);
  };
  auto hdr_load = [&](int32_t q) {
    return hdr_at(q < nbatch ? q : (nbatch > 0 ? nbatch - 1 : 0));
  };
  auto hdr = [](uint32_t hv, int k) { return (uint32_t)__builtin_amdgcn_readlane((int)hv, k); };
  uint32_t hv1 = hdr_at(wave);
  uint32_t hv2 = hdr_at(wave + NW);
  uint32_t w[6];
  {
    constexpr int U = 4;
    auto stage = [&](int32_t s) {
      int32_t c0[U], o0[U], sl[U];
      double v[U];
#pragma unroll
      for (int u = 0; u < U; ++u) {
        const int32_t q = s + u;
        c0[u] = sx[2 * q];
        o0[u] = sx[2 * q + 1];
        const int32_t on = sx[2 * q + 3];
        sl[u] = q < nseg ? ((q + 1 < nseg ? on : W) - o0[u]) : 0;
      }
#pragma unroll
      for (int u = 0; u < U; ++u) {
        const int32_t c = c0[u] + (lane < sl[u] ? lane : 0);
        v[u] = (c < n_local) ? x[c] : x_halo[c - n_local];
      }
#pragma unroll
      for (int u = 0; u < U; ++u)
        if (lane < sl[u]) xw[o0[u] + lane] = v[u];
    };
    for (int t = threadIdx.x; t < nd; t += 64 * NW) ds[t] = dict[doff + t];
    if (wave < nbatch && (int32_t)hdr(hv1, 1) < 0) vs_shared_fetch(hdr(hv1, 0), sbase, lane, w);
    stage(wave * U);
    for (int32_t s = (wave + NW) * U; s < nseg; s += NW * U) stage(s);
  }
  __syncthreads();
  const int q16 = lane >> 4;
  const int rsel = 4 * (2 * ((((q16 & 1) << 1) | (q16 >> 1)) + 4 * ((lane >> 3) & 1) + 8 * ((lane >> 2) & 1)) + 1);
  auto store = [&](double s, int32_t r, bool mine) {
    if (mine && r >= 0) {
      if (EPI == 0)
        y[r] = s;
      else if (EPI == 1)
        y[r] = fma(alpha, s, y[r]);
      else if (EPI == 2)
        y[r] = d[r] * s;
      else {
        y[r] = s;
        y2[r] = d[r] * s;
      }
    }
  };
  for (int32_t bi = wave; bi < nbatch; bi += NW) {
    uint32_t lo[16];
#pragma unroll
    for (int i = 0; i < 16; ++i) lo[i] = hdr(hv1, 2 * i);
    const bool shared = (int32_t)hdr(hv1, 1) < 0;
    const bool sixteen = shared && (int32_t)hdr(hv1, 17) >= 0;
    const bool eight = shared && !sixteen && (int32_t)hdr(hv1, 9) >= 0;
    const uint32_t eb = vs_off(lo[0]);
    const int cls = vs_cls(lo[0]);
    const int32_t full = cls > 0 ? 64 * (cls - 1) : 0;
    const uint8_t *fb = sbase + 16u * (size_t)eb;
    double sres;
    int mstep;
    uint32_t n0, n1;
    if (sixteen) {
      const int32_t rem = vs_len(lo[0]) - full;
      int32_t sh[16];
      sh[0] = 0;
// ... 237 lines not shown
```

### fictitious_domain_al_preconditioners_amd/solver.py

```python
from __future__ import annotations

import ctypes as C
import os

import numpy as np

from . import _abi

_HERE = os.path.dirname(os.path.abspath(__file__))
LIB_PATH = os.path.join(_HERE, "lib", "libalfd.so")
_lib = None

ABI_SYMBOLS = [
    "alfd_abi_version", "alfd_strerror", "alfd_last_error", "alfd_create", "alfd_destroy",
    "alfd_comm_unique_id", "alfd_comm_init", "alfd_set_partition", "alfd_set_matrix", "alfd_set_diag",
    "alfd_configure", "alfd_default_config", "alfd_setup", "alfd_precond_apply", "alfd_system_apply",
    "alfd_augment_rhs", "alfd_solve", "alfd_upload_rhs", "alfd_solve_resident", "alfd_download_solution",
    "alfd_get_history", "alfd_spmv", "alfd_dot", "alfd_matrix_lanes", "alfd_bench_spmv",
    "alfd_enable_timing", "alfd_get_timing", "alfd_host_halo_plan", "alfd_local_group_create",
    "alfd_local_group_destroy", "alfd_comm_init_local", "alfd_set_aggregates",
    "alfd_set_aggregate_partition", "alfd_get_matrix_info", "alfd_bench_spmv_format",
    "alfd_host_window_plan", "alfd_set_tunable", "alfd_build_aggregates", "alfd_get_aggregates",
    "alfd_host_aggregate_level", "alfd_comm_init_host",
    "alfd_get_device_memory", "alfd_set_row_blocks", "alfd_host_stream_plan",
    "alfd_host_row_blocks_from_points", "alfd_host_stream_plan_short", "alfd_set_prolongator", "alfd_set_controls", "alfd_get_timing_streamed", "alfd_get_setup_seconds",
    "alfd_host_numbering_from_points", "alfd_host_brick_blocks_from_points", "alfd_host_permute_csr",
    "alfd_build_smoothed_aggregation", "alfd_get_prolongator", "alfd_host_smoothed_prolongator",
    "alfd_build_smoothed_aggregation_truncated", "alfd_host_truncate_prolongator",
    "alfd_inner_prec_apply", "alfd_spmv_scaled",
    "alfd_estimate_spectrum", "alfd_get_cg_coefficients", "alfd_host_tridiagonal_extremes",
    "alfd_constraint_residual",
    "alfd_set_prolongator_block", "alfd_build_smoothed_aggregation_block", "alfd_get_prolongator_block",
    "alfd_clear_hierarchy", "alfd_get_inner_iterations", "alfd_get_aggregates_block",
    "alfd_host_strength_graph", "alfd_host_aggregate_graph", "alfd_build_strength_graph", "alfd_get_strength_graph",
]


class AlfdError(RuntimeError):

    def __init__(self, status, message):
        super().__init__(f"alfd status {status}: {message}")
        self.status = status


class NoConvergence(AlfdError):
    pass


def load_library():
    global _lib
    if _lib is not None:
        return _lib
    if not os.path.exists(LIB_PATH):
        raise ImportError(f"{LIB_PATH} is missing: the HIP extension is required (no CPU fallback). "
                          "Build it with `python -c 'import __graft_entry__ as g; g.build()'`.")
    lib = C.CDLL(LIB_PATH)
    vp, i32, i64, dbl = C.c_void_p, C.c_int32, C.c_int64, C.c_double
    PP = C.POINTER(C.c_void_p)
    sig = {
        "alfd_abi_version": (C.c_int, []),
        "alfd_strerror": (C.c_char_p, [C.c_int]),
        "alfd_last_error": (C.c_char_p, [vp]),
        "alfd_create": (C.c_int, [C.POINTER(vp), C.c_int]),
        "alfd_destroy": (C.c_int, [vp]),
        "alfd_comm_unique_id": (C.c_int, [vp, C.c_size_t]),
        "alfd_comm_init": (C.c_int, [vp, C.c_int, C.c_int, vp, C.c_size_t]),
        "alfd_set_partition": (C.c_int, [vp, C.c_int, PP]),
        "alfd_set_matrix": (C.c_int, [vp, C.c_int, i64, i64, vp, vp, vp]),
        "alfd_set_diag": (C.c_int, [vp, C.c_int, i64, vp]),
        "alfd_configure": (C.c_int, [vp, C.POINTER(_abi.Config)]),
        "alfd_default_config": (None, [C.POINTER(_abi.Config), C.c_int]),
        "alfd_setup": (C.c_int, [vp]),
        "alfd_precond_apply": (C.c_int, [vp, PP, PP, C.POINTER(_abi.Result)]),
        "alfd_system_apply": (C.c_int, [vp, PP, PP]),
        "alfd_augment_rhs": (C.c_int, [vp, PP]),
        "alfd_solve": (C.c_int, [vp, PP, PP, C.POINTER(_abi.Result)]),
        "alfd_upload_rhs": (C.c_int, [vp, PP, PP]),
        "alfd_solve_resident": (C.c_int, [vp, C.POINTER(_abi.Result)]),
        "alfd_download_solution": (C.c_int, [vp, PP]),
        "alfd_get_history": (C.c_int, [vp, vp, i32, C.POINTER(i32)]),
        "alfd_spmv": (C.c_int, [vp, C.c_int, vp, vp, C.c_int, dbl]),
        "alfd_spmv_scaled": (C.c_int, [vp, C.c_int, vp, vp, vp, vp]),
        "alfd_dot": (C.c_int, [vp, i64, vp, vp, C.POINTER(dbl)]),
        "alfd_inner_prec_apply": (C.c_int, [vp, C.c_int, vp, vp]),
        "alfd_matrix_lanes": (C.c_int, [vp, C.c_int, C.POINTER(i32)]),
        "alfd_bench_spmv": (C.c_int, [vp, C.c_int, i32, C.POINTER(dbl), C.POINTER(dbl)]),
        "alfd_enable_timing": (C.c_int, [vp, C.c_int]),
        "alfd_get_timing": (C.c_int, [vp, vp, vp, vp]),
        "alfd_host_halo_plan": (C.c_int, [i64, vp, vp, C.c_int, C.c_int, vp, vp, i64, C.POINTER(i64), vp]),
        "alfd_local_group_create": (C.c_int, [C.c_int, C.POINTER(vp)]),
        "alfd_local_group_destroy": (C.c_int, [vp]),
        "alfd_comm_init_local": (C.c_int, [vp, vp, C.c_int]),
        "alfd_set_aggregates": (C.c_int, [vp, C.c_int, i64, vp, vp, i64]),
        "alfd_set_aggregate_partition": (C.c_int, [vp, C.c_int, vp]),
        "alfd_set_prolongator": (C.c_int, [vp, C.c_int, i64, i64, vp, vp, vp]),
        "alfd_set_controls": (C.c_int, [vp, vp, vp, vp]),
        "alfd_get_timing_streamed": (C.c_int, [vp, vp]),
        "alfd_get_setup_seconds": (C.c_int, [vp, vp]),
        "alfd_get_matrix_info": (C.c_int, [vp, C.c_int, C.POINTER(_abi.MatrixInfo)]),
        "alfd_bench_spmv_format": (C.c_int, [vp, C.c_int, i32, C.c_int, C.POINTER(dbl), C.POINTER(dbl)]),
        "alfd_host_window_plan": (C.c_int, [i64, vp, vp, vp, i32, i32, C.POINTER(_abi.WindowPlanInfo)]),
        "alfd_set_tunable": (C.c_int, [vp, C.c_char_p, C.c_int]),
        "alfd_build_aggregates": (C.c_int, [vp, i32, dbl, i32, i64, i32, C.POINTER(i32)]),
        "alfd_get_aggregates": (C.c_int, [vp, C.c_int, vp, i64, C.POINTER(i64), C.POINTER(i64)]),
        "alfd_host_aggregate_level": (C.c_int, [i64, vp, vp, vp, i32, dbl, i32, vp, C.POINTER(i64)]),
        "alfd_build_smoothed_aggregation": (C.c_int, [vp, i32, dbl, i32, dbl, i64, i32, C.POINTER(i32), vp]),
        "alfd_build_smoothed_aggregation_truncated": (C.c_int, [vp, i32, dbl, i32, dbl, dbl, i32, i64, i32,
                                                                C.POINTER(i32), vp]),
        "alfd_host_truncate_prolongator": (C.c_int, [i64, i64, vp, vp, vp, vp, i32, dbl, i32, vp, vp, vp, i64,
                                                     C.POINTER(i64)]),
        "alfd_get_prolongator": (C.c_int, [vp, C.c_int, vp, vp, vp, i64, C.POINTER(i64), C.POINTER(i64),
                                           C.POINTER(i64)]),
        "alfd_host_smoothed_prolongator": (C.c_int, [i64, vp, vp, vp, i64, vp, vp, vp, vp, dbl, vp, i64, dbl,
                                                     vp, vp, vp, i64, C.POINTER(i64)]),
        "alfd_comm_init_host": (C.c_int, [vp, C.c_int, C.c_int, vp, vp, vp]),
        "alfd_get_device_memory": (C.c_int, [vp, C.POINTER(i64), C.POINTER(i64)]),
        "alfd_set_row_blocks": (C.c_int, [vp, C.c_int, i64, vp, vp]),
        "alfd_host_stream_plan": (C.c_int, [i64, vp, vp, vp, C.c_int32, i64, vp, vp, vp]),
        "alfd_host_row_blocks_from_points": (C.c_int, [i64, C.c_int32, vp, C.c_int32, vp, vp, vp]),
        "alfd_host_stream_plan_short": (C.c_int, [i64, vp, vp, vp, C.c_int32, vp]),
        "alfd_host_numbering_from_points": (C.c_int, [i64, C.c_int32, vp, vp]),
        "alfd_host_brick_blocks_from_points": (C.c_int, [i64, C.c_int32, vp, vp, C.c_int32, vp, vp, vp]),
        "alfd_host_permute_csr": (C.c_int, [i64, vp, vp, vp, vp, vp, vp, vp, vp]),
        "alfd_estimate_spectrum": (C.c_int, [vp, C.c_int, C.POINTER(_abi.Control), C.POINTER(_abi.Spectrum)]),
        "alfd_get_cg_coefficients": (C.c_int, [vp, vp, vp, i32, C.POINTER(i32)]),
        "alfd_host_tridiagonal_extremes": (C.c_int, [i32, vp, vp, C.POINTER(dbl), C.POINTER(dbl)]),
        "alfd_constraint_residual": (C.c_int, [vp, PP, vp, C.POINTER(dbl)]),
        "alfd_set_prolongator_block": (C.c_int, [vp, C.c_int, C.c_int, i64, i64, vp, vp, vp]),
        "alfd_build_smoothed_aggregation_block": (C.c_int, [vp, C.c_int, i32, dbl, i32, dbl, dbl, i32, i64, i32,
                                                            C.POINTER(i32), vp]),
        "alfd_get_prolongator_block": (C.c_int, [vp, C.c_int, C.c_int, vp, vp, vp, i64, C.POINTER(i64), C.POINTER(i64),
                                                 C.POINTER(i64)]),
        "alfd_clear_hierarchy": (C.c_int, [vp, C.c_int]),
        "alfd_get_aggregates_block": (C.c_int, [vp, C.c_int, C.c_int, vp, i64, C.POINTER(i64), C.POINTER(i64)]),
        "alfd_get_inner_iterations": (C.c_int, [vp, vp]),
        "alfd_host_strength_graph": (C.c_int, [i64, vp, vp, vp, i32, dbl, vp, vp, vp, vp, vp, i64, C.POINTER(i64)]),
        "alfd_host_aggregate_graph": (C.c_int, [i64, vp, vp, vp, vp, i32, i32, vp, C.POINTER(i64)]),
        "alfd_build_strength_graph": (C.c_int, [vp, i32, dbl, C.POINTER(i64), C.POINTER(i64)]),
        "alfd_get_strength_graph": (C.c_int, [vp, vp, vp, vp, vp, vp, i64, C.POINTER(i32)]),
    }
    for name, (res, args) in sig.items():
        fn = getattr(lib, name)
        fn.restype = res
        fn.argtypes = args
    _lib = lib
    return lib


def _blocks(arrs):
    a = (C.c_void_p * len(arrs))()
    for i, x in enumerate(arrs):
        a[i] = x.ctypes.data
    return a


class Context:

    def __init__(self, device_id=0):
        self._lib = load_library()
        self._h = C.c_void_p()
        rc = self._lib.alfd_create(C.byref(self._h), device_id)
        if rc != _abi.OK:
            self._h = None
            raise AlfdError(rc, "alfd_create failed: " + self._lib.alfd_strerror(rc).decode() +
                            " (a HIP device is required; there is no CPU path)")
# ... 157 lines not shown

    def _in(self, blocks):
        out = [np.ascontiguousarray(b, np.float64) for b in blocks]
        if [b.size for b in out] != self.block_sizes:
            raise ValueError(f"block sizes {[b.size for b in out]} != {self.block_sizes}")
        return out

    def precond_apply(self, src):
        src = self._in(src)
        dst = [np.zeros(n) for n in self.block_sizes]
        res = _abi.Result()
        self._ck(self._lib.alfd_precond_apply(self._h, _blocks(src), _blocks(dst), C.byref(res)))
        return dst, res

    def system_apply(self, src):
        src = self._in(src)
        dst = [np.zeros(n) for n in self.block_sizes]
        self._ck(self._lib.alfd_system_apply(self._h, _blocks(src), _blocks(dst)))
        return dst

    def augment_rhs(self, rhs):
        rhs = [b.copy() for b in self._in(rhs)]
        self._ck(self._lib.alfd_augment_rhs(self._h, _blocks(rhs)))
        return rhs

    def solve(self, rhs, x0=None, raise_on_failure=True):
        rhs = self._in(rhs)
        x = [np.zeros(n) for n in self.block_sizes] if x0 is None else [b.copy() for b in self._in(x0)]
        res = _abi.Result()
        rc = self._lib.alfd_solve(self._h, _blocks(rhs), _blocks(x), C.byref(res))
        if rc != _abi.OK and raise_on_failure:
            self._ck(rc)
        return x, res

    def upload_rhs(self, rhs, x0=None):
        rhs = self._in(rhs)
        x0_arrs = self._in(x0) if x0 is not None else None
        x0b = _blocks(x0_arrs) if x0_arrs is not None else None
        self._ck(self._lib.alfd_upload_rhs(self._h, _blocks(rhs), x0b))
        del x0_arrs

    def solve_resident(self, raise_on_failure=True):
        res = _abi.Result()
        rc = self._lib.alfd_solve_resident(self._h, C.byref(res))
        if rc != _abi.OK and raise_on_failure:
            self._ck(rc)
        return res

    def download_solution(self):
        x = [np.zeros(n) for n in self.block_sizes]
        self._ck(self._lib.alfd_download_solution(self._h, _blocks(x)))
        return x

    def history(self):
        cnt = C.c_int32(0)
        self._lib.alfd_get_history(self._h, None, 0, C.byref(cnt))
        out = np.zeros(max(cnt.value, 1))
        self._lib.alfd_get_history(self._h, out.ctypes.data, cnt.value, C.byref(cnt))
        return out[:cnt.value]

    def spmv(self, slot, x, y=None, mode=0, alpha=1.0):
        x = np.ascontiguousarray(x, np.float64)
        lanes = C.c_int32()
        self._ck(self._lib.alfd_matrix_lanes(self._h, slot, C.byref(lanes)))
        if y is None:
            raise ValueError("pass y (its length is the row count)")
        y = np.ascontiguousarray(y, np.float64).copy()
        self._ck(self._lib.alfd_spmv(self._h, slot, x.ctypes.data, y.ctypes.data, mode, alpha))
        return y, lanes.value

    def spmv_scaled(self, slot, x, d, y, y2=None):
        x = np.ascontiguousarray(x, np.float64)
        d = np.ascontiguousarray(d, np.float64)
        y = np.ascontiguousarray(y, np.float64).copy()
        if d.size != y.size or (y2 is not None and np.size(y2) != y.size):
            raise ValueError("d, y and y2 have the row count of the slot")
        if y2 is None:
            self._ck(self._lib.alfd_spmv_scaled(self._h, slot, x.ctypes.data, d.ctypes.data, y.ctypes.data, None))
            return y
        y2 = np.ascontiguousarray(y2, np.float64).copy()
        self._ck(self._lib.alfd_spmv_scaled(self._h, slot, x.ctypes.data, d.ctypes.data, y.ctypes.data, y2.ctypes.data))
        return y, y2

    def dot(self, x, y):
        x = np.ascontiguousarray(x, np.float64)
        y = np.ascontiguousarray(y, np.float64)
        out = C.c_double()
        self._ck(self._lib.alfd_dot(self._h, x.size, x.ctypes.data, y.ctypes.data, C.byref(out)))
        return out.value

    def inner_prec_apply(self, r, op=_abi.INNER_OP_AUG):
        r = np.ascontiguousarray(r, np.float64)
        bs = self.block_sizes
        if bs is None:
            n = r.size
        else:
            n = {_abi.INNER_OP_AUG: bs[0], _abi.INNER_OP_A22: bs[1]}.get(op, bs[0] + bs[1])
            if r.size != n:
                raise ValueError(f"r has {r.size} entries, the inner operator {n}")
        z = np.zeros(n)
        self._ck(self._lib.alfd_inner_prec_apply(self._h, int(op), r.ctypes.data, z.ctypes.data))
        return z

    def estimate_spectrum(self, op=_abi.SPECTRUM_CCT, control=None):
        out = _abi.Spectrum()
        self._ck(self._lib.alfd_estimate_spectrum(self._h, int(op), None if control is None else C.byref(control),
                                                  C.byref(out)))
        return out

    def cg_coefficients(self):
        cnt = C.c_int32(0)
        self._ck(self._lib.alfd_get_cg_coefficients(self._h, None, None, 0, C.byref(cnt)))
        alpha, beta = np.zeros(cnt.value), np.zeros(max(cnt.value, 1))
        self._ck(self._lib.alfd_get_cg_coefficients(self._h, alpha.ctypes.data, beta.ctypes.data, cnt.value,
                                                    C.byref(cnt)))
        return alpha, beta[:max(cnt.value - 1, 0)].copy()

    def constraint_residual(self, x, g=None):
        x = self._in(x)
        gv = None if g is None else np.ascontiguousarray(g, np.float64)
        if gv is not None and gv.size != self.block_sizes[-1]:
            raise ValueError(f"g has {gv.size} entries, the multiplier block {self.block_sizes[-1]}")
        out = C.c_double()
        self._ck(self._lib.alfd_constraint_residual(self._h, _blocks(x), None if gv is None else gv.ctypes.data,
                                                    C.byref(out)))
        return out.value

    def bench_spmv(self, slot, reps=20):
        ms, nbytes = C.c_double(), C.c_double()
        self._ck(self._lib.alfd_bench_spmv(self._h, slot, reps, C.byref(ms), C.byref(nbytes)))
        return ms.value, nbytes.value

    def bench_spmv_format(self, slot, reps=20, value_index=True):
        ms, nbytes = C.c_double(), C.c_double()
        self._ck(self._lib.alfd_bench_spmv_format(self._h, slot, reps, int(value_index), C.byref(ms),
                                                  C.byref(nbytes)))
        return ms.value, nbytes.value

    def matrix_info(self, slot):
        info = _abi.MatrixInfo()
        self._ck(self._lib.alfd_get_matrix_info(self._h, slot, C.byref(info)))
        return {k: getattr(info, k) for k, _ in info._fields_ if k != "reserved"}

    def set_tunable(self, name, value):
        self._ck(self._lib.alfd_set_tunable(self._h, name.encode(), int(value)))

    def set_row_blocks(self, slot, block_ptr, rows):
        if block_ptr is None:
            self._ck(self._lib.alfd_set_row_blocks(self._h, slot, 0, None, None))
            return
        bp = np.ascontiguousarray(block_ptr, np.int64)
        rw = np.ascontiguousarray(rows, np.int32)
        self._ck(self._lib.alfd_set_row_blocks(self._h, slot, bp.size - 1, bp.ctypes.data, rw.ctypes.data))

    def device_memory(self):
        f, t = C.c_int64(0), C.c_int64(0)
        self._ck(self._lib.alfd_get_device_memory(self._h, C.byref(f), C.byref(t)))
        return f.value, t.value

    def enable_timing(self, on=True):
        self._ck(self._lib.alfd_enable_timing(self._h, int(on)))

    def timing(self):
        ms = np.zeros(_abi.T_NCLASSES)
        n = np.zeros(_abi.T_NCLASSES, np.int64)
        b = np.zeros(_abi.T_NCLASSES)
# ... 441 lines not shown
```

### include/alfd/alfd.h

```cpp
#ifndef ALFD_H
#define ALFD_H

#include <stddef.h>
#include <stdint.h>

#ifdef __cplusplus
extern "C" {
#endif

#define ALFD_ABI_VERSION 12
#define ALFD_MAX_BLOCKS 3

enum alfd_status {
  ALFD_OK = 0,
  ALFD_E_INVALID = 1,
  ALFD_E_HIP = 2,
  ALFD_E_NO_CONVERGENCE_OUTER = 3,
  ALFD_E_NO_CONVERGENCE_INNER = 4,
  ALFD_E_BREAKDOWN = 5,
  ALFD_E_NOT_SETUP = 6,
  ALFD_E_COMM = 7,
  ALFD_E_UNSUPPORTED = 8
};

// ... 119 lines not shown
typedef int (*alfd_host_allgather_fn)(void *user, const void *send, void *recv, size_t bytes);
typedef int (*alfd_host_alltoallv_fn)(void *user, const void *send, const int64_t *send_off, void *recv,
                                      const int64_t *recv_off, size_t elem_size);
int alfd_comm_init_host(alfd_ctx_t ctx, int rank, int nranks, alfd_host_allgather_fn allgather,
                        alfd_host_alltoallv_fn alltoallv, void *user);

int alfd_host_halo_plan(int64_t nnz, const int32_t *col, const int64_t *col_offsets ,
                        int nranks, int rank, int32_t *col_local ,
                        int32_t *halo_globals , int64_t halo_capacity,
                        int64_t *n_halo, int64_t *recv_off );

int alfd_set_matrix(alfd_ctx_t ctx, int slot, int64_t nrows, int64_t ncols, const int64_t *row_ptr,
                    const int32_t *col, const double *val);
int alfd_set_diag(alfd_ctx_t ctx, int slot, int64_t n, const double *d);
#define ALFD_MAX_LEVELS 8
int alfd_set_aggregates(alfd_ctx_t ctx, int level, int64_t n_fine, const int32_t *agg, const double *weight,
                        int64_t n_coarse);
int alfd_set_prolongator(alfd_ctx_t ctx, int level, int64_t n_fine, int64_t n_coarse, const int64_t *row_ptr,
                         const int32_t *col, const double *val);
int alfd_set_aggregate_partition(alfd_ctx_t ctx, int level, const int64_t *coarse_offsets);
int alfd_build_aggregates(alfd_ctx_t ctx, int32_t block_size, double threshold, int32_t max_aggregate_nodes,
                          int64_t min_coarse, int32_t max_levels, int32_t *levels_out);
int alfd_get_aggregates(alfd_ctx_t ctx, int level, int32_t *agg, int64_t capacity, int64_t *n_fine,
                        int64_t *n_coarse);
int alfd_host_aggregate_level(int64_t nrows, const int64_t *row_ptr, const int32_t *col, const double *val,
                              int32_t block_size, double threshold, int32_t max_aggregate_nodes, int32_t *agg,
                              int64_t *n_coarse);
int alfd_host_strength_graph(int64_t nrows, const int64_t *row_ptr, const int32_t *col, const double *val,
                             int32_t block_size, double threshold, double *d, int32_t *fixed, int64_t *node_ptr,
                             int32_t *nbr, double *weight, int64_t capacity, int64_t *nnz);
int alfd_host_aggregate_graph(int64_t n_nodes, const int32_t *fixed, const int64_t *node_ptr, const int32_t *nbr,
                              const double *weight, int32_t block_size, int32_t max_aggregate_nodes, int32_t *agg,
                              int64_t *n_coarse);
int alfd_build_strength_graph(alfd_ctx_t ctx, int32_t block_size, double threshold, int64_t *n_nodes, int64_t *nnz);
int alfd_get_strength_graph(alfd_ctx_t ctx, double *d, int32_t *fixed, int64_t *node_ptr, int32_t *nbr, double *weight,
                            int64_t capacity, int32_t *on_device);
int alfd_build_smoothed_aggregation(alfd_ctx_t ctx, int32_t block_size, double threshold, int32_t max_aggregate_nodes,
                                    double damping, int64_t min_coarse, int32_t max_levels, int32_t *levels_out,
                                    double *omega_out);
int alfd_build_smoothed_aggregation_truncated(alfd_ctx_t ctx, int32_t block_size, double threshold,
                                              int32_t max_aggregate_nodes, double damping, double drop_tolerance,
                                              int32_t max_row_entries, int64_t min_coarse, int32_t max_levels,
                                              int32_t *levels_out, double *omega_out);
int alfd_get_prolongator(alfd_ctx_t ctx, int level, int64_t *row_ptr, int32_t *col, double *val, int64_t capacity,
                         int64_t *n_fine, int64_t *n_coarse, int64_t *nnz);
int alfd_set_prolongator_block(alfd_ctx_t ctx, int block, int level, int64_t n_fine, int64_t n_coarse,
                               const int64_t *row_ptr, const int32_t *col, const double *val);
int alfd_build_smoothed_aggregation_block(alfd_ctx_t ctx, int block, int32_t block_size, double threshold,
                                          int32_t max_aggregate_nodes, double damping, double drop_tolerance,
                                          int32_t max_row_entries, int64_t min_coarse, int32_t max_levels,
                                          int32_t *levels_out, double *omega_out);
int alfd_get_prolongator_block(alfd_ctx_t ctx, int block, int level, int64_t *row_ptr, int32_t *col, double *val,
                               int64_t capacity, int64_t *n_fine, int64_t *n_coarse, int64_t *nnz);
int alfd_get_aggregates_block(alfd_ctx_t ctx, int block, int level, int32_t *agg, int64_t capacity, int64_t *n_fine,
                              int64_t *n_coarse);
int alfd_clear_hierarchy(alfd_ctx_t ctx, int block);
int alfd_host_smoothed_prolongator(int64_t nrows, const int64_t *row_ptr, const int32_t *col, const double *val,
                                   int64_t n_mult, const int64_t *ct_row_ptr, const int32_t *ct_col, const double *ct_val,
                                   const double *w_inv, double gamma, const int32_t *agg, int64_t n_coarse, double omega,
                                   int64_t *p_row_ptr, int32_t *p_col, double *p_val, int64_t capacity, int64_t *nnz);
int alfd_host_truncate_prolongator(int64_t nrows, int64_t n_coarse, const int64_t *p_row_ptr, const int32_t *p_col,
                                   const double *p_val, const int32_t *agg, int32_t block_size, double drop_tolerance,
                                   int32_t max_row_entries, int64_t *out_row_ptr, int32_t *out_col, double *out_val,
                                   int64_t capacity, int64_t *nnz);
int alfd_configure(alfd_ctx_t ctx, const alfd_config *cfg);
int alfd_set_controls(alfd_ctx_t ctx, const alfd_control *outer, const alfd_control *inner, const alfd_control *mp_inner);
void alfd_default_config(alfd_config *cfg, int variant);
int alfd_setup(alfd_ctx_t ctx);

int alfd_precond_apply(alfd_ctx_t ctx, const double *const *src_blocks, double *const *dst_blocks,
                       alfd_result *res);
int alfd_system_apply(alfd_ctx_t ctx, const double *const *src_blocks, double *const *dst_blocks);
int alfd_augment_rhs(alfd_ctx_t ctx, double *const *rhs_blocks);
int alfd_solve(alfd_ctx_t ctx, const double *const *rhs_blocks, double *const *x_blocks,
               alfd_result *res);
int alfd_upload_rhs(alfd_ctx_t ctx, const double *const *rhs_blocks, const double *const *x0_blocks);
int alfd_solve_resident(alfd_ctx_t ctx, alfd_result *res);
int alfd_download_solution(alfd_ctx_t ctx, double *const *x_blocks);
int alfd_get_inner_iterations(alfd_ctx_t ctx, int64_t counts[3]);
int alfd_get_history(alfd_ctx_t ctx, double *out, int32_t capacity, int32_t *count);

int alfd_spmv(alfd_ctx_t ctx, int slot, const double *x, double *y, int mode, double alpha);
int alfd_spmv_scaled(alfd_ctx_t ctx, int slot, const double *x, const double *d, double *y, double *y2);
int alfd_dot(alfd_ctx_t ctx, int64_t n, const double *x, const double *y, double *result);
enum alfd_inner_op { ALFD_INNER_OP_AUG = 0, ALFD_INNER_OP_A22 = 1, ALFD_INNER_OP_AUG2 = 2 };
int alfd_inner_prec_apply(alfd_ctx_t ctx, int op, const double *r, double *z);
typedef struct alfd_spectrum {
  int32_t converged;
  int32_t steps;
  double initial_residual, last_residual;
  double lambda_min, lambda_max, condition;
} alfd_spectrum;
enum alfd_spectrum_op { ALFD_SPECTRUM_CCT = 0 };
int alfd_estimate_spectrum(alfd_ctx_t ctx, int op, const alfd_control *ctrl ,
                           alfd_spectrum *out);
int alfd_get_cg_coefficients(alfd_ctx_t ctx, double *alpha, double *beta, int32_t capacity, int32_t *count);
int alfd_host_tridiagonal_extremes(int32_t k, const double *alpha, const double *beta, double *lambda_min, double *lambda_max);
int alfd_constraint_residual(alfd_ctx_t ctx, const double *const *x_blocks, const double *g , double *linf);
int alfd_matrix_lanes(alfd_ctx_t ctx, int slot, int32_t *lanes);
int alfd_bench_spmv(alfd_ctx_t ctx, int slot, int32_t reps, double *ms_per_launch,
                    double *algorithmic_bytes);
typedef struct alfd_matrix_info {
  int32_t lanes, windowed, value_indexed;
  int32_t batch_major;
  int64_t nnz, window_blocks, window_fallback_blocks;
  int64_t value_indexed_blocks, value_indexed_nnz, dictionary_entries, value_wide_nnz;
  double algorithmic_bytes, streamed_bytes;
  int64_t shared_nnz;
  int64_t batch_major_blocks;
  int64_t batch_major_wide;
  int64_t batch_major_interior_blocks;
} alfd_matrix_info;
int alfd_get_matrix_info(alfd_ctx_t ctx, int slot, alfd_matrix_info *out);
typedef struct alfd_window_plan_info {
  int32_t windowed, value_indexed, row_block, max_window;
  int64_t blocks, fallback_blocks, segments;
  int64_t value_indexed_blocks, value_indexed_nnz, value_wide_nnz, dictionary_entries;
  int64_t batches, decode_mismatches;
} alfd_window_plan_info;
int alfd_host_window_plan(int64_t nrows, const int64_t *row_ptr, const int32_t *col, const double *val,
                          int32_t lanes, int32_t want_value_index, alfd_window_plan_info *out);
typedef struct alfd_stream_plan_info {
  int32_t ok, max_window, max_rows, max_batches;
  int64_t blocks, batches, segments, dictionary_entries, stream_bytes;
  int64_t decode_mismatches, rows_covered;
  int64_t shared_nnz;
} alfd_stream_plan_info;
int alfd_host_stream_plan(int64_t nrows, const int64_t *row_ptr, const int32_t *col, const double *val,
                          int32_t row_block, int64_t n_blocks, const int64_t *block_ptr, const int32_t *rows,
                          alfd_stream_plan_info *out);
int alfd_host_stream_plan_short(int64_t nrows, const int64_t *row_ptr, const int32_t *col, const double *val,
                                int32_t lanes, alfd_stream_plan_info *out);
int alfd_bench_spmv_format(alfd_ctx_t ctx, int slot, int32_t reps, int use_value_index,
                           double *ms_per_launch, double *streamed_bytes);
int alfd_set_row_blocks(alfd_ctx_t ctx, int slot, int64_t n_blocks, const int64_t *block_ptr, const int32_t *rows);

int alfd_host_row_blocks_from_points(int64_t nrows, int32_t dim, const double *points, int32_t max_rows,
                                     int64_t *n_blocks_out, int64_t *block_ptr_out, int32_t *rows_out);

int alfd_host_numbering_from_points(int64_t nrows, int32_t dim, const double *points, int64_t *new_to_old);
int alfd_host_brick_blocks_from_points(int64_t nrows, int32_t dim, const double *points, const int32_t *brick,
                                       int32_t max_rows, int64_t *n_blocks_out, int64_t *block_ptr_out, int32_t *rows_out);
int alfd_host_permute_csr(int64_t nrows, const int64_t *row_ptr, const int32_t *col, const double *val,
                          const int64_t *row_new_to_old, const int64_t *col_old_to_new, int64_t *out_row_ptr,
                          int32_t *out_col, double *out_val);

int alfd_get_device_memory(alfd_ctx_t ctx, int64_t *free_bytes, int64_t *total_bytes);
int alfd_set_tunable(alfd_ctx_t ctx, const char *name, int value);
enum alfd_timing_class {
  ALFD_T_SPMV_A = 0,
  ALFD_T_SPMV_OTHER = 1,
  ALFD_T_DOT = 2,
  ALFD_T_VEC = 3,
  ALFD_T_NCLASSES = 4
};
int alfd_enable_timing(alfd_ctx_t ctx, int on);
int alfd_get_timing(alfd_ctx_t ctx, double *ms , int64_t *launches ,
                    double *algorithmic_bytes );
int alfd_get_timing_streamed(alfd_ctx_t ctx, double *streamed_bytes );
enum alfd_setup_phase {
  ALFD_SETUP_UPLOAD = 0,
  ALFD_SETUP_DIAG_LAMBDA = 1,
  ALFD_SETUP_ML_FETCH = 2,
  ALFD_SETUP_ML_GALERKIN = 3,
  ALFD_SETUP_ML_UPLOAD = 4,
  ALFD_SETUP_ML_LAMBDA = 5,
// ... 11 lines not shown
```

Baseline: 15.04.

## Fuse A and C SpMVs into one paired launch on coarse levels

Adds a pair-launch mode where one grid runs the A SpMV blocks and then extra blocks that compute the W-scaled C SpMV (t = w*Cx) from the same input vector. The pair is used in the augmented operator and the multilevel correction, which removes one kernel launch per pair and lets both products run concurrently. The default ml_fuse is raised to 2, which enables pairing on coarse levels but not on the fine A. The kernels gain a template parameter and an extra argument, which may change register use and, through the xcd remap, block placement.

Result: faster. 15.65 (median of 6 runs) (+4.1%).

```diff
diff --git a/fictitious_domain_al_preconditioners_amd/csrc/alfd.hip b/fictitious_domain_al_preconditioners_amd/csrc/alfd.hip
--- a/fictitious_domain_al_preconditioners_amd/csrc/alfd.hip
+++ b/fictitious_domain_al_preconditioners_amd/csrc/alfd.hip
@@ -263,7 +263,7 @@
   int ml_rep_level = -1;
   bool dots_replicated = false;
   int64_t ml_rep_threshold = 300000;
-  int ml_fuse = 1;
+  int ml_fuse = 2;
   int ml_tail_rows = 0;
   int ml_gpu_galerkin = 1;
   double *g_w = nullptr, *g_tlam = nullptr;
@@ -537,7 +537,7 @@
   const int grid = (int)std::max<int64_t>(1, std::min<int64_t>((nbatches + 3) / 4, 256 * ctx->spmv_grid_mult));
 #define ALFD_STREAM(EPI)                                                                              \
   hipLaunchKernelGGL((spmv_stream_kernel<R, U, EPI, NT>), dim3(grid), dim3(kBlock), 0, ctx->stream,   \
-                     m.nrows, m.rp, m.col, m.val, x, m.halo, m.n_local_cols, y, alpha, d, y2)
+                     m.nrows, m.rp, m.col, m.val, x, m.halo, m.n_local_cols, y, alpha, d, y2, NoPair())
   if (epi == 0) ALFD_STREAM(0);
   else if (epi == 1) ALFD_STREAM(1);
   else if (epi == 2) ALFD_STREAM(2);
@@ -698,9 +698,7 @@
 #undef ALFD_VSS
 }
 
-static bool launch_vs(alfd_ctx *ctx, const DevCsr &m, const double *x, double *y, int epi, double alpha,
-                      const double *d, double *y2, int64_t first_block = 0, int64_t n_blocks = -1) {
-  const DevCsr::Vs &v = m.vs;
+static bool vs_lds_base_ok(alfd_ctx *ctx) {
   if (ctx->vs_lds_base_ok < 0) {
     uint32_t *probe = nullptr, base = 1;
     if (hipMalloc((void **)&probe, sizeof(uint32_t)) == hipSuccess) {
@@ -713,7 +711,13 @@
     if (!ctx->vs_lds_base_ok)
       std::fprintf(stderr, "[alfd] dynamic LDS does not start at offset 0 (%u): batch-major SpMV formats disabled\n", base);
   }
-  if (!ctx->vs_lds_base_ok) return false;
+  return ctx->vs_lds_base_ok != 0;
+}
+
+static bool launch_vs(alfd_ctx *ctx, const DevCsr &m, const double *x, double *y, int epi, double alpha,
+                      const double *d, double *y2, int64_t first_block = 0, int64_t n_blocks = -1) {
+  const DevCsr::Vs &v = m.vs;
+  if (!vs_lds_base_ok(ctx)) return false;
   if (v.L == 32) return launch_vss<32>(ctx, m, x, y, epi, alpha, d, y2), true;
   if (v.L == 16) return launch_vss<16>(ctx, m, x, y, epi, alpha, d, y2), true;
   if (v.L == 8) return launch_vss<8>(ctx, m, x, y, epi, alpha, d, y2), true;
@@ -724,7 +728,7 @@
   const unsigned grid = (unsigned)n_blocks;
   const int32_t base = (int32_t)first_block;
 #define ALFD_VS_ARGS \
-  v.stream, v.tab, v.stride, v.hdrb, v.segx, v.seg_stride, v.dict, x, m.halo, m.n_local_cols, y, alpha, d, y2, ctx->vs_xcd, base
+  v.stream, v.tab, v.stride, v.hdrb, v.segx, v.seg_stride, v.dict, x, m.halo, m.n_local_cols, y, alpha, d, y2, ctx->vs_xcd, base, NoPair()
 #define ALFD_VS(EPI, NWV)                                                                                        \
   do {                                                                                                           \
     if (v.wide)                                     \
@@ -858,6 +862,64 @@
   return spmv_m(ctx, m, slot == ALFD_A ? ALFD_T_SPMV_A : ALFD_T_SPMV_OTHER, x, y, epi, alpha, d, y2);
 }
 
+static bool tail_form(const DevCsr &m) { return m.present && !m.vs.on && !m.win; }
+
+
+static int pair_form_A(alfd_ctx *ctx, const DevCsr &A) {
+  if (!A.present || A.sparse || A.n_list == 0) return 0;
+  if (A.vs.on && ctx->vs_enable && !ctx->vi_off)
+    return A.vs.L == 64 && !A.vs.wide && ctx->vs_NW == 4 && A.vs.nb > 0 && vs_lds_base_ok(ctx) ? 1 : 0;
+  if (A.win) return 0;
+  return A.L == 64 && ctx->spmv_stream_R == 2 && ctx->spmv_stream_U == 8 && !ctx->spmv_nt ? 2 : 0;
+}
+
+static inline bool gd_nested(const alfd_ctx *ctx);
+static int pair_forms(alfd_ctx *ctx, const DevCsr &A, const DevCsr &C) {
+  const bool ok = ctx->nranks == 1 && ctx->cfg.w_inverse == ALFD_W_DIAGONAL && !ctx->cfg.aug_assembled && !gd_nested(ctx) &&
+                  tail_form(C) && !C.sparse && C.nrows > 0 && (C.L == 16 || C.L == 32 || C.L == 64) && A.ncols == C.ncols;
+  return ok ? pair_form_A(ctx, A) : 0;
+}
+static int pair_ok(alfd_ctx *ctx, const DevCsr &A, const DevCsr &C) {
+  const bool fine = &A == &ctx->mat[ALFD_A] || &A == &ctx->mat[ALFD_A2];
+  return ctx->ml_fuse >= (fine ? 3 : 2) ? pair_forms(ctx, A, C) : 0;
+}
+
+static int launch_pair(alfd_ctx *ctx, int form, const DevCsr &A, int clsA, const DevCsr &C, const double *w,
+                       const double *x, double *y, double *t) {
+  const bool vi = !ctx->vi_off, vs = ctx->vs_enable != 0 && !ctx->vi_off;
+  Timer tm(ctx, clsA, A.algorithmic_bytes() + C.algorithmic_bytes(), A.streamed_bytes(vi, vs) + C.streamed_bytes(vi, vs));
+  PairC pc;
+  pc.nrows = C.n_list, pc.rp = C.rp, pc.col = C.col, pc.val = C.val, pc.x_halo = C.halo, pc.d = w, pc.t = t;
+  pc.n_local = C.n_local_cols, pc.L = C.L;
+  pc.nC = (uint32_t)grid_for_rows(C.n_list, C.L);
+  if (form == 1) {
+    const DevCsr::Vs &v = A.vs;
+    const size_t lds = (size_t)VsFmt<0>::kWinOff + (size_t)v.maxW * sizeof(double);
+    pc.nA = (uint32_t)v.nb;
+#define ALFD_VS_PAIR(TAG)                                                                                                  \
+  hipLaunchKernelGGL((spmv_vs_kernel<0, TAG, 4, 0, true>), dim3(pc.nA + pc.nC), dim3(256), lds, ctx->stream, v.stream,    \
+                     v.tab, v.stride, v.hdrb, v.segx, v.seg_stride, v.dict, x, A.halo, A.n_local_cols, y, 0.0,            \
+                     (const double *)nullptr, (double *)nullptr, ctx->vs_xcd, 0, pc)
+    if (A.tag == 0) ALFD_VS_PAIR(0);
+    else ALFD_VS_PAIR(1);
+#undef ALFD_VS_PAIR
+  } else {
+    const int64_t nbatches = (A.nrows + 1) / 2;
+    pc.nA = (uint32_t)std::max<int64_t>(1, std::min<int64_t>((nbatches + 3) / 4, 256 * ctx->spmv_grid_mult));
+    hipLaunchKernelGGL((spmv_stream_kernel<2, 8, 0, false, true>), dim3(pc.nA + pc.nC), dim3(kBlock), 0, ctx->stream,
+                       A.nrows, A.rp, A.col, A.val, x, A.halo, A.n_local_cols, y, 0.0, (const double *)nullptr,
+                       (double *)nullptr, pc);
+  }
+  HIPC(hipGetLastError());
+  return ALFD_OK;
+}
+
+static int spmv_AC(alfd_ctx *ctx, DevCsr &A, int clsA, DevCsr &C, const double *w, const double *x, double *y, double *t) {
+  if (const int form = pair_ok(ctx, A, C)) return launch_pair(ctx, form, A, clsA, C, w, x, y, t);
+  RC(spmv_m(ctx, A, clsA, x, y, 0));
+  return spmv_m(ctx, C, ALFD_T_SPMV_OTHER, x, t, 2, 0.0, w);
+}
+
 static int finish_dots(alfd_ctx *ctx, int64_t nb, int count, int out, int fin) {
   if (ctx->nranks == 1 || ctx->dots_replicated) {
     hipLaunchKernelGGL(dot_final_kernel, dim3(count), dim3(kBlock), 0, ctx->stream, ctx->partial, nb,
@@ -927,13 +989,14 @@
   const double *w = ctx->diag[ALFD_INVW];
   switch (op) {
     case OP_AUG:
-      RC(spmv(ctx, ALFD_A, x, y, 0));
-      if (ctx->cfg.aug_assembled) return ALFD_OK;
+      if (ctx->cfg.aug_assembled) return spmv(ctx, ALFD_A, x, y, 0);
       if (exact_w && ctx->cfg.w_inverse != ALFD_W_DIAGONAL) {
+        RC(spmv(ctx, ALFD_A, x, y, 0));
         RC(spmv(ctx, ALFD_C, x, ctx->t_lam, 0));
         RC(winv_scale(ctx, 1.0, ctx->t_lam, ctx->t_lam));
       } else {
-        RC(spmv(ctx, ALFD_C, x, ctx->t_lam, 2, 0.0, w));
+        if (!ctx->mat[ALFD_A].present || !ctx->mat[ALFD_C].present) return ctx->err = "matrix not set", ALFD_E_NOT_SETUP;
+        RC(spmv_AC(ctx, ctx->mat[ALFD_A], ALFD_T_SPMV_A, ctx->mat[ALFD_C], w, x, y, ctx->t_lam));
       }
       RC(spmv(ctx, ALFD_CT, ctx->t_lam, y, 1, ctx->cfg.gamma));
       if (!gd_nested(ctx)) return ALFD_OK;
@@ -3501,8 +3564,7 @@
 }
 
 static int fused_AC(alfd_ctx *ctx, const AugOp &F, const double *x, double *y) {
-  RC(spmv_m(ctx, *F.A, F.clsA, x, y, 0));
-  return spmv_m(ctx, *F.C, ALFD_T_SPMV_OTHER, x, F.tlam, 2, 0.0, F.w);
+  return spmv_AC(ctx, *F.A, F.clsA, *F.C, F.w, x, y, F.tlam);
 }
 
 static int aug_apply(alfd_ctx *ctx, const AugOp &F, const double *x, double *y) {
@@ -3619,8 +3681,6 @@
 }
 
 static_assert(kTailMaxLevels == ALFD_MAX_LEVELS + 1, "TailTable holds every level of a hierarchy");
-
-static bool tail_form(const DevCsr &m) { return m.present && !m.vs.on && !m.win; }
 
 static TailCsr tail_csr(const DevCsr &m) {
   TailCsr t;
@@ -3796,15 +3856,12 @@
   }
   RC(ml_cycle(ctx, 0, 0, Q.rr, z));
   hipLaunchKernelGGL(scatter_add_kernel, dim3(gm), dim3(256), 0, ctx->stream, Q.m, Q.S, Q.zS, z);
-  RC(spmv_m(ctx, Q.As, ALFD_T_SPMV_OTHER, z, Q.uS, 0));
+  if (pen) RC(spmv_AC(ctx, Q.As, ALFD_T_SPMV_OTHER, ctx->mat[ALFD_C], w, z, Q.uS, ctx->t_lam));
+  else RC(spmv_m(ctx, Q.As, ALFD_T_SPMV_OTHER, z, Q.uS, 0));
   if (fused_ok(ctx, F)) {
-    RC(spmv(ctx, ALFD_C, z, ctx->t_lam, 2, 0.0, w));
     RC(fused_correct(ctx, F, pdeg, pratio, Q.rS, Q.uS, Q.eS, nullptr));
   } else {
-    if (pen) {
-      RC(spmv(ctx, ALFD_C, z, ctx->t_lam, 2, 0.0, w));
-      RC(spmv_m(ctx, Q.Cts, ALFD_T_SPMV_OTHER, ctx->t_lam, Q.uS, 1, ctx->cfg.gamma));
-    }
+    if (pen) RC(spmv_m(ctx, Q.Cts, ALFD_T_SPMV_OTHER, ctx->t_lam, Q.uS, 1, ctx->cfg.gamma));
     VEC_LAUNCH(sub_from_kernel, Q.mpad, 24, Q.rS, Q.uS);
     RC(aug_cheb(ctx, F, pdeg, pratio, Q.uS, Q.eS));
   }
@@ -6218,7 +6275,7 @@
   if (const char *e = std::getenv("ALFD_SPMV_WINDOW_MAXW")) ctx->win_maxW = std::min(16384, std::max(256, std::atoi(e)));
   if (const char *e = std::getenv("ALFD_ML_REPLICATE")) ctx->ml_rep_threshold = std::atoll(e);
   if (const char *e = std::getenv("ALFD_ML_GPU_GALERKIN")) ctx->ml_gpu_galerkin = std::atoi(e);
-  if (const char *e = std::getenv("ALFD_ML_FUSE")) ctx->ml_fuse = std::atoi(e) != 0;
+  if (const char *e = std::getenv("ALFD_ML_FUSE")) ctx->ml_fuse = std::max(0, std::min(3, std::atoi(e)));
   if (const char *e = std::getenv("ALFD_SPMV_VI_LEVELS")) ctx->vi_levels = std::atoi(e);
   if (const char *e = std::getenv("ALFD_SPMV_BATCH_MAJOR")) ctx->vs_enable = std::atoi(e);
   if (const char *e = std::getenv("ALFD_SPMV_BATCH_MAJOR_ROWS")) ctx->vs_RB = std::max(4, std::min(kVsMaxRows, std::atoi(e)));
@@ -7359,6 +7416,36 @@
   return rc;
 }
 
+int alfd_spmv_pair(alfd_ctx_t ctx, int slot_a, int slot_c, const double *x, const double *d, double *y, double *t) {
+  CHECK_CTX();
+  for (int slot : {slot_a, slot_c})
+    if (slot < 0 || slot >= ALFD_NSLOTS || !ctx->mat[slot].present) return ALFD_E_INVALID;
+  if (!x || !d || !y || !t || t == y) return ALFD_E_INVALID;
+  const DevCsr &A = ctx->mat[slot_a], &Cm = ctx->mat[slot_c];
+  const int form = pair_forms(ctx, A, Cm);
+  if (!form) return ctx->err = "alfd_spmv_pair: the two slots do not qualify for the pair launch", ALFD_E_UNSUPPORTED;
+  double *dx = nullptr, *dd = nullptr, *dy = nullptr, *dt = nullptr;
+  HIPC(hipMalloc((void **)&dx, A.ncols * sizeof(double)));
+  HIPC(hipMalloc((void **)&dd, Cm.nrows * sizeof(double)));
+  HIPC(hipMalloc((void **)&dy, A.nrows * sizeof(double)));
+  HIPC(hipMalloc((void **)&dt, Cm.nrows * sizeof(double)));
+  HIPC(hipMemcpyAsync(dx, x, A.ncols * sizeof(double), hipMemcpyHostToDevice, ctx->stream));
+  HIPC(hipMemcpyAsync(dd, d, Cm.nrows * sizeof(double), hipMemcpyHostToDevice, ctx->stream));
+  HIPC(hipMemcpyAsync(dy, y, A.nrows * sizeof(double), hipMemcpyHostToDevice, ctx->stream));
+  HIPC(hipMemcpyAsync(dt, t, Cm.nrows * sizeof(double), hipMemcpyHostToDevice, ctx->stream));
+  const int rc = launch_pair(ctx, form, A, slot_a == ALFD_A ? ALFD_T_SPMV_A : ALFD_T_SPMV_OTHER, Cm, dd, dx, dy, dt);
+  if (rc == ALFD_OK) {
+    HIPC(hipMemcpyAsync(y, dy, A.nrows * sizeof(double), hipMemcpyDeviceToHost, ctx->stream));
+    HIPC(hipMemcpyAsync(t, dt, Cm.nrows * sizeof(double), hipMemcpyDeviceToHost, ctx->stream));
+    HIPC(hipStreamSynchronize(ctx->stream));
+  }
+  hipFree(dx);
+  hipFree(dd);
+  hipFree(dy);
+  hipFree(dt);
+  return rc;
+}
+
 int alfd_inner_prec_apply(alfd_ctx_t ctx, int op, const double *r, double *z) {
   CHECK_CTX();
   CHECK_SETUP();
@@ -7993,7 +8080,7 @@
     return ALFD_OK;
   }
   if (std::strcmp(name, "ml_fuse") == 0) {
-    ctx->ml_fuse = value != 0;
+    ctx->ml_fuse = std::max(0, std::min(3, value));
     return ALFD_OK;
   }
   if (std::strcmp(name, "ml_tail_rows") == 0) {
diff --git a/fictitious_domain_al_preconditioners_amd/csrc/kernels.hpp b/fictitious_domain_al_preconditioners_amd/csrc/kernels.hpp
--- a/fictitious_domain_al_preconditioners_amd/csrc/kernels.hpp
+++ b/fictitious_domain_al_preconditioners_amd/csrc/kernels.hpp
@@ -1,6 +1,7 @@
 #pragma once
 #include <hip/hip_runtime.h>
 #include <stdint.h>
+#include <type_traits>
 
 namespace alfd {
 
@@ -149,20 +150,17 @@
 }
 
 template <int L, int EPI, bool SPARSE>
-__global__ __launch_bounds__(kBlock) void spmv_kernel(int64_t nrows, const int64_t *__restrict__ rp,
-                                                      const int32_t *__restrict__ col,
-                                                      const double *__restrict__ val,
-                                                      const int32_t *__restrict__ rows,
-                                                      const double *__restrict__ x,
-                                                      const double *__restrict__ x_halo, int32_t n_local,
-                                                      double *__restrict__ y, double alpha,
-                                                      const double *__restrict__ d,
-                                                      double *__restrict__ y2) {
+__device__ __forceinline__ void spmv_rows(int64_t block, int64_t nblocks, int64_t nrows,
+                                          const int64_t *__restrict__ rp, const int32_t *__restrict__ col,
+                                          const double *__restrict__ val, const int32_t *__restrict__ rows,
+                                          const double *__restrict__ x, const double *__restrict__ x_halo,
+                                          int32_t n_local, double *__restrict__ y, double alpha,
+                                          const double *__restrict__ d, double *__restrict__ y2) {
   constexpr int RPB = kBlock / L;
   const int lane = threadIdx.x % L;
   const int sub = threadIdx.x / L;
   const int64_t ngroups = (nrows + RPB - 1) / RPB;
-  for (int64_t g = blockIdx.x; g < ngroups; g += gridDim.x) {
+  for (int64_t g = block; g < ngroups; g += nblocks) {
     const int64_t r = g * RPB + sub;
     if (r < nrows) {
       const int64_t k0 = rp[r], k1 = rp[r + 1];
@@ -190,16 +188,58 @@
   }
 }
 
-template <int R, int U, int EPI, bool NT>
+template <int L, int EPI, bool SPARSE>
+__global__ __launch_bounds__(kBlock) void spmv_kernel(int64_t nrows, const int64_t *__restrict__ rp,
+                                                      const int32_t *__restrict__ col,
+                                                      const double *__restrict__ val,
+                                                      const int32_t *__restrict__ rows,
+                                                      const double *__restrict__ x,
+                                                      const double *__restrict__ x_halo, int32_t n_local,
+                                                      double *__restrict__ y, double alpha,
+                                                      const double *__restrict__ d,
+                                                      double *__restrict__ y2) {
+  spmv_rows<L, EPI, SPARSE>(blockIdx.x, gridDim.x, nrows, rp, col, val, rows, x, x_halo, n_local, y, alpha, d, y2);
+}
+
+struct PairC {
+  int64_t nrows;
+  const int64_t *rp;
+  const int32_t *col;
+  const double *val, *x_halo, *d;
+  double *t;
+  int32_t n_local, L;
+  uint32_t nA, nC;
+};
+struct NoPair {};
+
+__device__ __forceinline__ uint32_t pair_nA(const NoPair &) { return gridDim.x; }
+__device__ __forceinline__ uint32_t pair_nA(const PairC &c) { return c.nA; }
+
+__device__ __forceinline__ bool pair_rows(const NoPair &, const double *) { return false; }
+__device__ __forceinline__ bool pair_rows(const PairC &c, const double *__restrict__ x) {
+  if (blockIdx.x < c.nA) return false;
+  const int64_t block = blockIdx.x - c.nA;
+  switch (c.L) {
+    case 16: spmv_rows<16, 2, false>(block, c.nC, c.nrows, c.rp, c.col, c.val, nullptr, x, c.x_halo, c.n_local, c.t, 0.0, c.d, nullptr); break;
+    case 32: spmv_rows<32, 2, false>(block, c.nC, c.nrows, c.rp, c.col, c.val, nullptr, x, c.x_halo, c.n_local, c.t, 0.0, c.d, nullptr); break;
+    default: spmv_rows<64, 2, false>(block, c.nC, c.nrows, c.rp, c.col, c.val, nullptr, x, c.x_halo, c.n_local, c.t, 0.0, c.d, nullptr); break;
+  }
+  return true;
+}
+template <bool PAIR>
+using PairArg = typename std::conditional<PAIR, PairC, NoPair>::type;
+
+template <int R, int U, int EPI, bool NT, bool PAIR = false>
 __global__ __launch_bounds__(kBlock) void spmv_stream_kernel(
     int64_t nrows, const int64_t *__restrict__ rp, const int32_t *__restrict__ col,
     const double *__restrict__ val, const double *__restrict__ x, const double *__restrict__ x_halo,
     int32_t n_local, double *__restrict__ y, double alpha, const double *__restrict__ d,
-    double *__restrict__ y2) {
+    double *__restrict__ y2, PairArg<PAIR> pc) {
+  if (pair_rows(pc, x)) return;
   const int lane = threadIdx.x & 63;
   const int wave = __builtin_amdgcn_readfirstlane(threadIdx.x >> 6);
   const int64_t nbatches = (nrows + R - 1) / R;
-  for (int64_t b = (int64_t)blockIdx.x * 4 + wave; b < nbatches; b += (int64_t)gridDim.x * 4) {
+  for (int64_t b = (int64_t)blockIdx.x * 4 + wave; b < nbatches; b += (int64_t)pair_nA(pc) * 4) {
     const int64_t r0 = b * R;
     int64_t kb[R + 1];
 #pragma unroll
diff --git a/fictitious_domain_al_preconditioners_amd/csrc/kernels_vs.hpp b/fictitious_domain_al_preconditioners_amd/csrc/kernels_vs.hpp
--- a/fictitious_domain_al_preconditioners_amd/csrc/kernels_vs.hpp
+++ b/fictitious_domain_al_preconditioners_amd/csrc/kernels_vs.hpp
@@ -112,13 +112,15 @@
   }
 }
 
-template <int EPI, int TAG, int NW, int WD = 0>
+template <int EPI, int TAG, int NW, int WD = 0, bool PAIR = false>
 __global__ __launch_bounds__(64 * NW) __attribute__((amdgpu_waves_per_eu(8, 8))) void spmv_vs_kernel(
     const uint8_t *__restrict__ stream, const uint64_t *__restrict__ tab, int32_t stride,
     const int32_t *__restrict__ hdrb, const int32_t *__restrict__ segx, int32_t seg_stride,
     const double *__restrict__ dict, const double *__restrict__ x, const double *__restrict__ x_halo,
     int32_t n_local, double *__restrict__ y, double alpha, const double *__restrict__ d, double *__restrict__ y2,
-    int xcd_remap, int32_t block_base) {
+    int xcd_remap, int32_t block_base, PairArg<PAIR> pc) {
+  static_assert(!PAIR || NW == 4, "the second party runs on kBlock threads");
+  if (pair_rows(pc, x)) return;
   extern __shared__ double xs[];
   char *sm = (char *)xs;
   double *ds = (double *)(sm + kVsDictOff);
@@ -127,7 +129,7 @@
   const int wave = __builtin_amdgcn_readfirstlane(threadIdx.x >> 6);
   int64_t b = blockIdx.x;
   if (xcd_remap) {
-    const int64_t nwg = gridDim.x, q = nwg / 8, rm = nwg % 8, xcd = b % 8, idx = b / 8;
+    const int64_t nwg = pair_nA(pc), q = nwg / 8, rm = nwg % 8, xcd = b % 8, idx = b / 8;
     b = (xcd < rm ? xcd * (q + 1) : rm * (q + 1) + (xcd - rm) * q) + idx;
   }
   b += block_base;
diff --git a/fictitious_domain_al_preconditioners_amd/solver.py b/fictitious_domain_al_preconditioners_amd/solver.py
--- a/fictitious_domain_al_preconditioners_amd/solver.py
+++ b/fictitious_domain_al_preconditioners_amd/solver.py
@@ -27,7 +27,7 @@
     "alfd_host_numbering_from_points", "alfd_host_brick_blocks_from_points", "alfd_host_permute_csr",
     "alfd_build_smoothed_aggregation", "alfd_get_prolongator", "alfd_host_smoothed_prolongator",
     "alfd_build_smoothed_aggregation_truncated", "alfd_host_truncate_prolongator",
-    "alfd_inner_prec_apply", "alfd_spmv_scaled",
+    "alfd_inner_prec_apply", "alfd_spmv_scaled", "alfd_spmv_pair",
     "alfd_estimate_spectrum", "alfd_get_cg_coefficients", "alfd_host_tridiagonal_extremes",
     "alfd_constraint_residual",
     "alfd_set_prolongator_block", "alfd_build_smoothed_aggregation_block", "alfd_get_prolongator_block",
@@ -81,6 +81,7 @@
         "alfd_get_history": (C.c_int, [vp, vp, i32, C.POINTER(i32)]),
         "alfd_spmv": (C.c_int, [vp, C.c_int, vp, vp, C.c_int, dbl]),
         "alfd_spmv_scaled": (C.c_int, [vp, C.c_int, vp, vp, vp, vp]),
+        "alfd_spmv_pair": (C.c_int, [vp, C.c_int, C.c_int, vp, vp, vp, vp]),
         "alfd_dot": (C.c_int, [vp, i64, vp, vp, C.POINTER(dbl)]),
         "alfd_inner_prec_apply": (C.c_int, [vp, C.c_int, vp, vp]),
         "alfd_matrix_lanes": (C.c_int, [vp, C.c_int, C.POINTER(i32)]),
@@ -404,6 +405,17 @@
         self._ck(self._lib.alfd_spmv_scaled(self._h, slot, x.ctypes.data, d.ctypes.data, y.ctypes.data, y2.ctypes.data))
         return y, y2
 
+    def spmv_pair(self, slot_a, slot_c, x, d, y, t):
+        x = np.ascontiguousarray(x, np.float64)
+        d = np.ascontiguousarray(d, np.float64)
+        y = np.ascontiguousarray(y, np.float64).copy()
+        t = np.ascontiguousarray(t, np.float64).copy()
+        if d.size != t.size:
+            raise ValueError("d and t have the row count of slot_c")
+        self._ck(self._lib.alfd_spmv_pair(self._h, slot_a, slot_c, x.ctypes.data, d.ctypes.data, y.ctypes.data,
+                                          t.ctypes.data))
+        return y, t
+
     def dot(self, x, y):
         x = np.ascontiguousarray(x, np.float64)
         y = np.ascontiguousarray(y, np.float64)
diff --git a/include/alfd/alfd.h b/include/alfd/alfd.h
--- a/include/alfd/alfd.h
+++ b/include/alfd/alfd.h
@@ -225,6 +225,7 @@
 
 int alfd_spmv(alfd_ctx_t ctx, int slot, const double *x, double *y, int mode, double alpha);
 int alfd_spmv_scaled(alfd_ctx_t ctx, int slot, const double *x, const double *d, double *y, double *y2);
+int alfd_spmv_pair(alfd_ctx_t ctx, int slot_a, int slot_c, const double *x, const double *d, double *y, double *t);
 int alfd_dot(alfd_ctx_t ctx, int64_t n, const double *x, const double *y, double *result);
 enum alfd_inner_op { ALFD_INNER_OP_AUG = 0, ALFD_INNER_OP_A22 = 1, ALFD_INNER_OP_AUG2 = 2 };
 int alfd_inner_prec_apply(alfd_ctx_t ctx, int op, const double *r, double *z);
diff --git a/profiles/pair_launch/families.py b/profiles/pair_launch/families.py
--- /dev/null
+++ b/profiles/pair_launch/families.py
@@ -0,0 +1,43 @@
+import csv
+import re
+import sys
+
+ARMS = ["parent", "fuse1", "fuse2", "fuse3"]
+FAMILIES = [
+    ("spmv_vs_kernel<0,0,4,0> (fine A)", r"spmv_vs_kernel<0, 0, 4, 0(, false)?>"),
+    ("spmv_vs_kernel<0,0,4,0,true> (fine A + C)", r"spmv_vs_kernel<0, 0, 4, 0, true>"),
+    ("spmv_vs_kernel<0,1,4,0> (patch, levels 1-2)", r"spmv_vs_kernel<0, 1, 4, 0(, false)?>"),
+    ("spmv_vs_kernel<0,1,4,0,true> (the same + C)", r"spmv_vs_kernel<0, 1, 4, 0, true>"),
+    ("spmv_stream_kernel<2,8,0> (levels 3-4)", r"spmv_stream_kernel<2, 8, 0, false(, false)?>"),
+    ("spmv_stream_kernel<2,8,0,.,true> (the same + C)", r"spmv_stream_kernel<2, 8, 0, false, true>"),
+    ("spmv_stream_kernel<2,8,2> (C, 64 lanes)", r"spmv_stream_kernel<2, 8, 2, false(, false)?>"),
+    ("spmv_kernel<16,2> (C)", r"spmv_kernel<16, 2, false>"),
+    ("spmv_kernel<32,2> (C)", r"spmv_kernel<32, 2, false>"),
+    ("aug_tail_kernel<*,*>", r"aug_tail_kernel<"),
+]
+
+
+def load(arm):
+    with open(f"{arm}_kernel_stats.csv") as f:
+        return [(r["Name"], int(r["Calls"]), int(r["TotalDurationNs"])) for r in csv.DictReader(f)]
+
+
+def main():
+    data = {a: load(a) for a in ARMS}
+    solves = 2.0
+    print("| family | " + " | ".join(f"{a} calls | ms | avg µs" for a in ARMS) + " |")
+    print("|---|" + "---|" * (3 * len(ARMS)))
+    for label, pat in FAMILIES:
+        cells = []
+        for a in ARMS:
+            rows = [(c, ns) for n, c, ns in data[a] if re.search(pat, n)]
+            calls, ns = sum(c for c, _ in rows), sum(t for _, t in rows)
+            cells.append(f"{calls / solves:.0f} | {ns / solves * 1e-6:.1f} | {ns / calls * 1e-3:.1f}" if calls else "0 | 0 | –")
+        print(f"| `{label}` | " + " | ".join(cells) + " |")
+    for a in ARMS:
+        calls = sum(c for _, c, _ in data[a])
+        print(f"{a}: {calls} kernel launches in the whole run", file=sys.stderr)
+
+
+if __name__ == "__main__":
+    main()
```
